# kwea123/nerf_pl

Hardware: AMD Instinct MI355X
Metric: rays/sec (64+128 samples), full training step: render_rays fwd + MSE + bwd + grad all-reduce + Adam (higher is better)
Workload: dtype bf16

## Files before the change

include/nerfhip.h:

```cpp
#ifndef NERFHIP_H
#define NERFHIP_H

#include <stddef.h>
#include <stdint.h>

#ifdef __cplusplus
extern "C" {
#endif

#define NERFHIP_ABI_VERSION 3

#define NERFHIP_E_BADARG (-1)
#define NERFHIP_E_UNSUPPORTED (-2)
#define NERFHIP_E_ALIGN (-3)
#define NERFHIP_E_DATA (-4)

#define NERFHIP_F32 0
#define NERFHIP_BF16 1
#define NERFHIP_BF16_F8 2

typedef void* nerfhip_stream_t;

int nerfhip_abi_version(void);
const char* nerfhip_error_string(int code);

int nerfhip_posenc(const float* x, float* out, int64_t n, int C, int n_freqs, nerfhip_stream_t stream);
int nerfhip_posenc_bwd(const float* x, const float* gout, float* gx, int64_t n, int C, int n_freqs,
                       nerfhip_stream_t stream);

int nerfhip_posenc_bands(const float* x, const float* bands, float* out, int64_t n, int C, int n_freqs,
                         nerfhip_stream_t stream);
int nerfhip_posenc_bands_bwd(const float* x, const float* bands, const float* gout, float* gx, int64_t n, int C, int n_freqs,
                             nerfhip_stream_t stream);

int nerfhip_sample_coarse_z(const float* rays, const float* perturb_rand, float* z, int64_t B, int S,
                            int use_disp, float perturb, nerfhip_stream_t stream);

int nerfhip_searchsorted_right(const float* a, const float* v, int64_t* idx, int64_t B, int M, int K,
                               nerfhip_stream_t stream);
int nerfhip_searchsorted_left(const float* a, const float* v, int64_t* idx, int64_t B, int M, int K,
                              nerfhip_stream_t stream);

int nerfhip_sample_pdf(const float* bins, int64_t bins_stride, const float* weights, int64_t w_stride,
                       const float* u, int64_t u_stride, float* samples, int64_t B, int M, int K, float eps,
                       nerfhip_stream_t stream);

#define NERFHIP_ROW_TOTAL_EXACT 0
#define NERFHIP_ROW_TOTAL_ATEN 1

int nerfhip_sample_pdf_ex(const float* bins, int64_t bins_stride, const float* weights, int64_t w_stride,
                          const float* u, int64_t u_stride, float* samples, int64_t B, int M, int K, float eps,
                          float* cdf_out, int64_t* inds_out, int row_total, nerfhip_stream_t stream);

int nerfhip_fine_z(const float* z_coarse, const float* w_coarse, const float* u, int64_t u_stride,
                   float* z_fine, float* z_new, int64_t B, int S_c, int N_i, float eps,
                   nerfhip_stream_t stream);

int nerfhip_fine_z_ex(const float* z_coarse, const float* w_coarse, const float* u, int64_t u_stride, float* z_fine,
                      float* z_new, int64_t B, int S_c, int N_i, float eps, float* cdf_out, int64_t* inds_out,
                      int row_total, nerfhip_stream_t stream);

int nerfhip_composite_fwd(const float* raw, int raw_ch, const float* z, const float* rays,
                          const float* noise, float noise_std, int white_back, float* weights, float* rgb,
                          float* depth, float* opacity, int64_t B, int S, nerfhip_stream_t stream);
int nerfhip_composite_bwd(const float* raw, int raw_ch, const float* z, const float* rays,
                          const float* noise, float noise_std, int white_back, const float* g_rgb,
                          const float* g_depth, const float* g_opacity, const float* g_weights,
                          float* g_raw, int64_t B, int S, nerfhip_stream_t stream);

int nerfhip_composite_train(const float* raw, const float* z, const float* rays, const float* noise, float noise_std,
                            int white_back, const float* target, float grad_scale, float* weights, float* rgb, float* depth,
                            float* opacity, float* g_raw, int64_t B, int S, nerfhip_stream_t stream);

int nerfhip_composite_train_fine_z(const float* raw, const float* z, const float* rays, const float* noise, float noise_std,
                                   int white_back, const float* target, float grad_scale, float* weights, float* rgb, float* depth,
                                   float* opacity, float* g_raw, int64_t B, int S, const float* u, int64_t u_stride, int N_i,
                                   float eps, float* z_fine, int row_total, nerfhip_stream_t stream);
int nerfhip_composite_train_loss(const float* raw, const float* z, const float* rays, const float* noise, float noise_std,
                                 int white_back, const float* target, float grad_scale, float* weights, float* rgb, float* depth,
                                 float* opacity, float* g_raw, int64_t B, int S, const float* rgb_coarse, float* out3,
                                 uint32_t* ticket, nerfhip_stream_t stream);

size_t nerfhip_mlp_packed_bytes(int dtype);
int nerfhip_mlp_pack_weights(const float* const* weights_host, const float* const* biases_host, void* packed,
                             int dtype, nerfhip_stream_t stream);

size_t nerfhip_mlp_act_bytes(int64_t n_points, int dtype);

int nerfhip_mlp_fwd_embedded(const float* x, int64_t x_stride, int64_t n, const void* packed, float* out,
                             int sigma_only, int dtype, void* save_acts, nerfhip_stream_t stream);

int nerfhip_mlp_fwd_rays(const float* rays, const float* z, int64_t B, int S, const void* packed, float* out,
                         int sigma_only, int dtype, void* save_acts, nerfhip_stream_t stream);

int nerfhip_mlp_fwd_rays_coarse(const float* rays, const float* perturb_rand, float* z, int64_t B, int S, int use_disp,
                                float perturb, const void* packed, float* out, int sigma_only, int dtype, void* save_acts,
                                nerfhip_stream_t stream);

size_t nerfhip_mlp_packed_bwd_bytes(int dtype);
int nerfhip_mlp_pack_weights_bwd(const float* const* weights_host, const float* const* biases_host, void* packed_bwd, int dtype,
                                 nerfhip_stream_t stream);
int nerfhip_mlp_pack_weights_train(const float* const* weights_host, const float* const* biases_host, void* packed,
                                   void* packed_bwd, int dtype, nerfhip_stream_t stream);
int nerfhip_mlp_pack_weights_train_multi(const float* const* weights_host, const float* const* biases_host,
                                         void* const* packed_host, void* const* packed_bwd_host, int n_models, int dtype,
                                         nerfhip_stream_t stream);
size_t nerfhip_mlp_dy_bytes(int64_t n_points, int dtype);
int nerfhip_mlp_dw_splits(int64_t n_points, int dtype);
size_t nerfhip_mlp_dw_workspace_bytes(int64_t n_points, int dtype);
int nerfhip_mlp_bwd(const float* g_out, const float* out, int64_t n, const void* packed_bwd, const void* acts,
                    void* dys, void* dw_workspace, float* const* grad_w_host, float* const* grad_b_host,
                    int accumulate, int dtype, nerfhip_stream_t stream);

int nerfhip_mlp_bwd_phases(const float* g_out, const float* out, int64_t n, const void* packed_bwd, const void* acts,
                           void* dys, void* dw_workspace, float* const* grad_w_host, float* const* grad_b_host,
                           int accumulate, int dtype, int phases, nerfhip_stream_t stream);

typedef struct nerfhip_adam_fused {
    int n_models;
    float* param[2];
    float* exp_avg[2];
    float* exp_avg_sq[2];
    const float* grad_flat[2];
    float* state;
    float lr, beta1, beta2, eps, weight_decay;
} nerfhip_adam_fused;
size_t nerfhip_mlp_dw_workspace_bytes_multi(const int64_t* n_points_host, int n_models, int dtype);
int nerfhip_mlp_dw_plan(const int64_t* n_points_host, int n_models, int dtype, int* splits_out, int* stage_kib_out);
int nerfhip_mlp_bwd_multi(int n_models, const float* const* g_out_host, const float* const* out_host, const int64_t* n_host,
                          const void* const* packed_bwd_host, const void* const* acts_host, void* const* dys_host,
                          void* dw_workspace, float* const* grad_w_host, float* const* grad_b_host, int accumulate, int dtype,
                          int phases, const float* g_scale, const nerfhip_adam_fused* adam, nerfhip_stream_t stream);

typedef struct nerfhip_enc_source {
    const float* rays[2];
    const float* z[2];
    int S[2];
} nerfhip_enc_source;
int nerfhip_mlp_bwd_multi_rays(int n_models, const float* const* g_out_host, const float* const* out_host, const int64_t* n_host,
                               const void* const* packed_bwd_host, const void* const* acts_host, void* const* dys_host,
                               void* dw_workspace, float* const* grad_w_host, float* const* grad_b_host, int accumulate, int dtype,
                               int phases, const float* g_scale, const nerfhip_adam_fused* adam, const nerfhip_enc_source* enc,
                               nerfhip_stream_t stream);

int nerfhip_mlp_dx_embedded(const void* dys, int64_t n, const float* w_xyz1, const float* w_xyz5, const float* w_dir,
                            float* gx, int64_t gx_stride, int dtype, nerfhip_stream_t stream);

#define NERFHIP_ACT_NONE 0
#define NERFHIP_ACT_RELU 1
#define NERFHIP_ACT_SIGMOID 2
int nerfhip_linear_fwd(const float* x, int64_t ldx, const float* w, int64_t ldw, const float* bias, float* y, int64_t ldy,
                       int64_t n, int n_in, int n_out, int act, int accumulate, int dtype, nerfhip_stream_t stream);
int nerfhip_linear_bwd_input(const float* gy, int64_t ldgy, const float* y, int64_t ldy, int act, const float* w, int64_t ldw,
                             float* gx, int64_t ldgx, int64_t n, int n_in, int n_out, int accumulate, int dtype,
                             nerfhip_stream_t stream);
size_t nerfhip_linear_bwd_weight_workspace_bytes(int64_t n, int n_in, int n_out);
int nerfhip_linear_bwd_weight(const float* gy, int64_t ldgy, const float* y, int64_t ldy, int act, const float* x, int64_t ldx,
                              float* gw, int64_t ldgw, float* gb, void* workspace, int64_t n, int n_in, int n_out,
                              int accumulate, int dtype, nerfhip_stream_t stream);

int nerfhip_mse_psnr(const float* rgb_coarse, const float* rgb_fine, const float* target, int64_t n, float* out3,
                     float* g_coarse, float* g_fine, nerfhip_stream_t stream);

int nerfhip_adam_step(float* const* params_host, const float* const* grads_host, float* const* exp_avg_host,
                      float* const* exp_avg_sq_host, const int64_t* numel_host, int n_tensors, float* state, float lr,
                      float beta1, float beta2, float eps, float weight_decay, nerfhip_stream_t stream);

int nerfhip_radam_step(float* const* params_host, const float* const* grads_host, float* const* exp_avg_host,
                       float* const* exp_avg_sq_host, const int64_t* numel_host, int n_tensors, float* state, double lr,
                       double beta1, double beta2, double eps, double weight_decay, int degenerated_to_sgd,
                       nerfhip_stream_t stream);
int nerfhip_ranger_step(float* const* params_host, const float* const* grads_host, float* const* exp_avg_host,
                        float* const* exp_avg_sq_host, const int64_t* numel_host, int n_tensors, float* state,
                        float* const* slow_host, double alpha, int k, double n_sma_threshold, double lr, double beta1,
                        double beta2, double eps, double weight_decay, nerfhip_stream_t stream);

int nerfhip_ray_directions(float* dirs, int H, int W, double focal, nerfhip_stream_t stream);
int nerfhip_get_rays(const float* directions, const float* c2w, float* rays_o, float* rays_d, int64_t n,
                     nerfhip_stream_t stream);
int nerfhip_ndc_rays(int H, int W, double focal, float near, const float* rays_o, const float* rays_d, float* out_o,
                     float* out_d, int64_t n, nerfhip_stream_t stream);
int nerfhip_gen_rays(const float* c2w, const int64_t* pixel_ids, int64_t first_pixel, int64_t n, int H, int W,
                     double focal, float near, float far, int use_ndc, float ndc_near_plane, float* rays,
                     nerfhip_stream_t stream);
int nerfhip_sample_batch(const float* c2w, const int64_t* pixel_ids, const float* rgbs_all, int64_t n, int H, int W,
                         double focal, float near, float far, int use_ndc, float ndc_near_plane, float* rays, float* rgbs,
                         nerfhip_stream_t stream);

#define NERFHIP_DRAW_UNIFORM 0
#define NERFHIP_DRAW_NORMAL 1
#define NERFHIP_DRAW_RANDINT 2
typedef struct nerfhip_draw {
    int kind;
    int64_t numel;
    void* out;
    uint64_t range;
} nerfhip_draw;
typedef struct nerfhip_ray_batch {
    const float* c2w;
    const float* rgbs_all;
    float* rays;
    float* rgbs;
    int H, W;
    double focal;
    float near, far;
    int use_ndc;
    float ndc_near_plane;
} nerfhip_ray_batch;
uint64_t nerfhip_torch_draw_increment(int64_t numel, int max_blocks);
int nerfhip_torch_draws(const nerfhip_draw* draws_host, int n_draws, const nerfhip_ray_batch* batch_host, uint64_t seed,
                        uint64_t offset, uint64_t* state, int max_blocks, uint64_t* increment_host, nerfhip_stream_t stream);

int nerfhip_train_prologue(const nerfhip_draw* draws_host, int n_draws, const nerfhip_ray_batch* batch_host, uint64_t seed,
                           uint64_t offset, uint64_t* state, int max_blocks, uint64_t* increment_host,
                           const float* const* weights_host, const float* const* biases_host, void* const* packed_host,
                           void* const* packed_bwd_host, int n_models, int dtype, nerfhip_stream_t stream);

typedef struct nerfhip_render_args {
    const float* rays;
    int64_t B;
    int S_c, N_i;
    const void* packed_coarse;
    const void* packed_fine;
    float* z_coarse;
    float* raw_coarse;
    float* z_fine;
    float* raw_fine;
    void* save_coarse;
    void* save_fine;
    const float* perturb_rand;
    float perturb;
    int use_disp;
    const float* noise_coarse;
    const float* noise_fine;
    float noise_std;
    int white_back;
    const float* u;
    int64_t u_stride;
    float eps;
    int row_total;
    float* rgb_coarse;
    float* depth_coarse;
    float* opacity_coarse;
    float* rgb_fine;
    float* depth_fine;
    float* opacity_fine;
    const float* target;
    float grad_scale;
    float* g_raw_coarse;
    float* g_raw_fine;
    float* out3;
    uint32_t* ticket;
    int regen_enc;
} nerfhip_render_args;
int nerfhip_render_supported(int64_t B, int S_c, int N_i, int dtype);
int nerfhip_render_fwd(const nerfhip_render_args* args_host, int dtype, nerfhip_stream_t stream);
int nerfhip_render_test_fwd(const nerfhip_render_args* args_host, int dtype, nerfhip_stream_t stream);
int nerfhip_render_train_fwd(const nerfhip_render_args* args_host, int dtype, nerfhip_stream_t stream);

size_t nerfhip_marching_cubes_workspace_bytes(int64_t n0, int64_t n1, int64_t n2);
int nerfhip_marching_cubes_count(const float* volume, int64_t n0, int64_t n1, int64_t n2, double iso, void* workspace,
                                 int64_t* totals, nerfhip_stream_t stream);
int nerfhip_marching_cubes_emit(const float* volume, int64_t n0, int64_t n1, int64_t n2, double iso, void* workspace,
                                const int64_t* totals, double* vertices, int32_t* triangles, nerfhip_stream_t stream);

int nerfhip_mesh_edge_keys(const int32_t* triangles, int64_t T, int64_t* keys, nerfhip_stream_t stream);
size_t nerfhip_mesh_cluster_workspace_bytes(int64_t V, int64_t T);
int nerfhip_mesh_largest_cluster(const int32_t* triangles, int64_t V, int64_t T, const int64_t* sorted_keys, const int64_t* order,
                                 void* workspace, int64_t* totals, nerfhip_stream_t stream);
int nerfhip_mesh_cluster_compact(const int32_t* triangles, int64_t V, int64_t T, void* workspace, int64_t* kept_vertex_ids,
                                 int32_t* kept_triangles, nerfhip_stream_t stream);

int nerfhip_mesh_vertex_normals(const float* vertices, int64_t V, const int32_t* triangles, int64_t T, double* normals,
                                nerfhip_stream_t stream);
int nerfhip_mesh_normal_rays(const float* vertices, const double* normals, int64_t V, float near, float far, float near_t,
                             float* rays, nerfhip_stream_t stream);
int nerfhip_mesh_view_rays(const float* vertices, int64_t V, const float* w2c_host, const float* origin_host, float focal, int W,
                           int H, const uint8_t* image, float near, uint8_t* colors, double* depth, float* rays,
                           nerfhip_stream_t stream);
int nerfhip_mesh_color_accumulate(const uint8_t* colors, const double* depth, const float* opacity, int64_t V,
                                  float occ_threshold, double* accum, nerfhip_stream_t stream);
int nerfhip_mesh_color_finish(const double* accum, int64_t V, uint8_t* out, nerfhip_stream_t stream);
int nerfhip_mesh_rgb_to_u8(const float* rgb, int64_t n, uint8_t* out, nerfhip_stream_t stream);

size_t nerfhip_vol_workspace_bytes(int64_t n);
int nerfhip_vol_pack(const float* rgbsigma, int64_t n, int64_t first_index, float neg_cell, void* workspace, uint32_t* records,
                     int64_t capacity, int64_t* cursor, nerfhip_stream_t stream);

int nerfhip_png_unfilter(const uint8_t* streams, uint8_t* out, int32_t* error_flags, int n_images, int H, int W, int ch,
                         nerfhip_stream_t stream);
int nerfhip_resize_rgba_lanczos(const uint8_t* in, uint8_t* out, uint8_t* workspace, int n_images, int in_h, int in_w, int out_h,
                                int out_w, const int32_t* xmin_h, const int32_t* count_h, const int32_t* taps_h, int ksize_h,
                                const int32_t* xmin_v, const int32_t* count_v, const int32_t* taps_v, int ksize_v,
                                nerfhip_stream_t stream);
int nerfhip_rgba_to_rgb_white(const uint8_t* rgba, float* rgb, uint8_t* valid_mask, int64_t n, nerfhip_stream_t stream);

int nerfhip_jpeg_entropy_decode(const uint8_t* scan, int64_t scan_bytes, int n_comp, const int32_t* comp, const uint8_t* huffman,
                                int huffman_mask, int mcus_x, int mcus_y, int restart_interval, int16_t* const* coef,
                                const int64_t* coef_blocks);
size_t nerfhip_jpeg_planes_bytes(int H, int W, int n_comp, int hs, int vs);
int nerfhip_jpeg_decode(const int16_t* coef_y, const int16_t* coef_cb, const int16_t* coef_cr, const uint16_t* quant,
                        uint8_t* planes, uint8_t* out, int n_images, int H, int W, int n_comp, int hs, int vs,
                        nerfhip_stream_t stream);

#define NERFHIP_IMAGE_PLANAR 0
#define NERFHIP_IMAGE_INTERLEAVED 1
size_t nerfhip_ssim_workspace_bytes(int B, int C, int H, int W);
int nerfhip_ssim(const float* img1, const float* img2, int B, int C, int H, int W, int window_size, int layout, float* map,
                 float* mean, void* workspace, nerfhip_stream_t stream);
size_t nerfhip_depth_colormap_workspace_bytes(int64_t n);
int nerfhip_depth_colormap(const float* depth, int64_t n, const uint8_t* table, float* out_chw, uint8_t* out_hwc, void* workspace,
                           nerfhip_stream_t stream);

#define NERFHIP_GIF_STRIP 3838
size_t nerfhip_gif_workspace_bytes(int F, int H, int W);
size_t nerfhip_gif_data_stride(int H, int W);
int nerfhip_gif_quantize(const uint8_t* frames, int F, int H, int W, uint8_t* indices, uint8_t* palettes, int32_t* box_counts,
                         void* workspace, nerfhip_stream_t stream);
int nerfhip_gif_lzw(const uint8_t* indices, int F, int H, int W, uint8_t* data, int32_t* lengths, void* workspace,
                    nerfhip_stream_t stream);

#define NERFHIP_PNG_STRIP 8192
size_t nerfhip_png_workspace_bytes(int n, int64_t stream_bytes);
size_t nerfhip_png_data_stride(int64_t stream_bytes);
int nerfhip_png_filter(const uint8_t* images, int n, int H, int W, int C, uint8_t* streams, nerfhip_stream_t stream);
int nerfhip_png_deflate(const uint8_t* streams, int n, int64_t stream_bytes, uint8_t* data, int32_t* lengths, uint32_t* adler,
                        void* workspace, nerfhip_stream_t stream);
int nerfhip_png_code_lengths(const uint32_t* counts, int n_symbols, int limit, uint8_t* lengths);

#ifdef __cplusplus
}
#endif
#endif
```

nerf_pl_amd/_lib.py:

```python
import ctypes
import functools
import os

import torch

_PKG = os.path.dirname(os.path.abspath(__file__))
LIB_PATH = os.environ.get("NERFHIP_LIB_PATH") or os.path.join(_PKG, "libnerfhip.so")

F32, BF16, BF16_F8 = 0, 1, 2

_c_void_p = ctypes.c_void_p
_i64 = ctypes.c_int64
_int = ctypes.c_int
_f32 = ctypes.c_float
_f64 = ctypes.c_double

SIGNATURES = {
    "nerfhip_abi_version": [],
    "nerfhip_error_string": [_int],
    "nerfhip_posenc": [_c_void_p, _c_void_p, _i64, _int, _int, _c_void_p],
    "nerfhip_posenc_bwd": [_c_void_p, _c_void_p, _c_void_p, _i64, _int, _int, _c_void_p],
    "nerfhip_posenc_bands": [_c_void_p, _c_void_p, _c_void_p, _i64, _int, _int, _c_void_p],
    "nerfhip_posenc_bands_bwd": [_c_void_p, _c_void_p, _c_void_p, _c_void_p, _i64, _int, _int, _c_void_p],
    "nerfhip_sample_coarse_z": [_c_void_p, _c_void_p, _c_void_p, _i64, _int, _int, _f32, _c_void_p],
    "nerfhip_searchsorted_right": [_c_void_p, _c_void_p, _c_void_p, _i64, _int, _int, _c_void_p],
    "nerfhip_searchsorted_left": [_c_void_p, _c_void_p, _c_void_p, _i64, _int, _int, _c_void_p],
    "nerfhip_sample_pdf": [_c_void_p, _i64, _c_void_p, _i64, _c_void_p, _i64, _c_void_p, _i64, _int, _int, _f32,
                           _c_void_p],
    "nerfhip_sample_pdf_ex": [_c_void_p, _i64, _c_void_p, _i64, _c_void_p, _i64, _c_void_p, _i64, _int, _int, _f32,
                              _c_void_p, _c_void_p, _int, _c_void_p],
    "nerfhip_fine_z_ex": [_c_void_p, _c_void_p, _c_void_p, _i64, _c_void_p, _c_void_p, _i64, _int, _int, _f32,
                          _c_void_p, _c_void_p, _int, _c_void_p],
    "nerfhip_fine_z": [_c_void_p, _c_void_p, _c_void_p, _i64, _c_void_p, _c_void_p, _i64, _int, _int, _f32,
                       _c_void_p],
    "nerfhip_composite_fwd": [_c_void_p, _int, _c_void_p, _c_void_p, _c_void_p, _f32, _int, _c_void_p, _c_void_p,
                              _c_void_p, _c_void_p, _i64, _int, _c_void_p],
    "nerfhip_composite_bwd": [_c_void_p, _int, _c_void_p, _c_void_p, _c_void_p, _f32, _int, _c_void_p, _c_void_p,
                              _c_void_p, _c_void_p, _c_void_p, _i64, _int, _c_void_p],
    "nerfhip_mlp_packed_bytes": [_int],
    "nerfhip_mlp_pack_weights": [ctypes.POINTER(_c_void_p), ctypes.POINTER(_c_void_p), _c_void_p, _int, _c_void_p],
    "nerfhip_mlp_act_bytes": [_i64, _int],
    "nerfhip_mlp_fwd_embedded": [_c_void_p, _i64, _i64, _c_void_p, _c_void_p, _int, _int, _c_void_p, _c_void_p],
    "nerfhip_mlp_fwd_rays": [_c_void_p, _c_void_p, _i64, _int, _c_void_p, _c_void_p, _int, _int, _c_void_p, _c_void_p],
    "nerfhip_mlp_packed_bwd_bytes": [_int],
    "nerfhip_mlp_pack_weights_bwd": [ctypes.POINTER(_c_void_p), ctypes.POINTER(_c_void_p), _c_void_p, _int, _c_void_p],
    "nerfhip_mlp_pack_weights_train": [ctypes.POINTER(_c_void_p), ctypes.POINTER(_c_void_p), _c_void_p, _c_void_p, _int, _c_void_p],
    "nerfhip_mlp_dy_bytes": [_i64, _int],
    "nerfhip_mlp_dw_splits": [_i64, _int],
    "nerfhip_mlp_dw_workspace_bytes": [_i64, _int],
    "nerfhip_ray_directions": [_c_void_p, _int, _int, ctypes.c_double, _c_void_p],
    "nerfhip_get_rays": [_c_void_p, _c_void_p, _c_void_p, _c_void_p, _i64, _c_void_p],
    "nerfhip_ndc_rays": [_int, _int, ctypes.c_double, _f32, _c_void_p, _c_void_p, _c_void_p, _c_void_p, _i64, _c_void_p],
    "nerfhip_gen_rays": [_c_void_p, _c_void_p, _i64, _i64, _int, _int, ctypes.c_double, _f32, _f32, _int, _f32, _c_void_p,
                         _c_void_p],
    "nerfhip_mse_psnr": [_c_void_p, _c_void_p, _c_void_p, _i64, _c_void_p, _c_void_p, _c_void_p, _c_void_p],
    "nerfhip_mlp_bwd_phases": [_c_void_p, _c_void_p, _i64, _c_void_p, _c_void_p, _c_void_p, _c_void_p,
                               ctypes.POINTER(_c_void_p), ctypes.POINTER(_c_void_p), _int, _int, _int, _c_void_p],
    "nerfhip_mlp_dx_embedded": [_c_void_p, _i64, _c_void_p, _c_void_p, _c_void_p, _c_void_p, _i64, _int, _c_void_p],
    "nerfhip_adam_step": [ctypes.POINTER(_c_void_p), ctypes.POINTER(_c_void_p), ctypes.POINTER(_c_void_p),
                          ctypes.POINTER(_c_void_p), ctypes.POINTER(_i64), _int, _c_void_p, _f32, _f32, _f32, _f32, _f32, _c_void_p],
    "nerfhip_radam_step": [ctypes.POINTER(_c_void_p), ctypes.POINTER(_c_void_p), ctypes.POINTER(_c_void_p),
                           ctypes.POINTER(_c_void_p), ctypes.POINTER(_i64), _int, _c_void_p, _f64, _f64, _f64, _f64, _f64, _int, _c_void_p],
    "nerfhip_ranger_step": [ctypes.POINTER(_c_void_p), ctypes.POINTER(_c_void_p), ctypes.POINTER(_c_void_p),
                            ctypes.POINTER(_c_void_p), ctypes.POINTER(_i64), _int, _c_void_p, ctypes.POINTER(_c_void_p), _f64, _int,
                            _f64, _f64, _f64, _f64, _f64, _f64, _c_void_p],
    "nerfhip_mlp_bwd": [_c_void_p, _c_void_p, _i64, _c_void_p, _c_void_p, _c_void_p, _c_void_p,
                        ctypes.POINTER(_c_void_p), ctypes.POINTER(_c_void_p), _int, _int, _c_void_p],
    "nerfhip_sample_batch": [_c_void_p, _c_void_p, _c_void_p, _i64, _int, _int, ctypes.c_double, _f32, _f32, _int, _f32, _c_void_p,
                             _c_void_p, _c_void_p],
    "nerfhip_mlp_pack_weights_train_multi": [ctypes.POINTER(_c_void_p), ctypes.POINTER(_c_void_p), ctypes.POINTER(_c_void_p),
                                             ctypes.POINTER(_c_void_p), _int, _int, _c_void_p],
    "nerfhip_render_supported": [_i64, _int, _int, _int],
    "nerfhip_render_test_fwd": [_c_void_p, _int, _c_void_p],
    "nerfhip_render_fwd": [_c_void_p, _int, _c_void_p],
    "nerfhip_render_train_fwd": [_c_void_p, _int, _c_void_p],
    "nerfhip_composite_train": [_c_void_p, _c_void_p, _c_void_p, _c_void_p, _f32, _int, _c_void_p, _f32, _c_void_p, _c_void_p,
                                _c_void_p, _c_void_p, _c_void_p, _i64, _int, _c_void_p],
    "nerfhip_composite_train_fine_z": [_c_void_p, _c_void_p, _c_void_p, _c_void_p, _f32, _int, _c_void_p, _f32, _c_void_p, _c_void_p,
                                       _c_void_p, _c_void_p, _c_void_p, _i64, _int, _c_void_p, _i64, _int, _f32, _c_void_p, _int, _c_void_p],
    "nerfhip_composite_train_loss": [_c_void_p, _c_void_p, _c_void_p, _c_void_p, _f32, _int, _c_void_p, _f32, _c_void_p, _c_void_p,
                                     _c_void_p, _c_void_p, _c_void_p, _i64, _int, _c_void_p, _c_void_p, _c_void_p, _c_void_p],
    "nerfhip_mlp_fwd_rays_coarse": [_c_void_p, _c_void_p, _c_void_p, _i64, _int, _int, _f32, _c_void_p, _c_void_p, _int, _int,
                                    _c_void_p, _c_void_p],
    "nerfhip_torch_draw_increment": [_i64, _int],
    "nerfhip_torch_draws": [_c_void_p, _int, _c_void_p, ctypes.c_uint64, ctypes.c_uint64, _c_void_p, _int,
                            ctypes.POINTER(ctypes.c_uint64), _c_void_p],
    "nerfhip_train_prologue": [_c_void_p, _int, _c_void_p, ctypes.c_uint64, ctypes.c_uint64, _c_void_p, _int,
                               ctypes.POINTER(ctypes.c_uint64), ctypes.POINTER(_c_void_p), ctypes.POINTER(_c_void_p),
                               ctypes.POINTER(_c_void_p), ctypes.POINTER(_c_void_p), _int, _int, _c_void_p],
    "nerfhip_mlp_dw_workspace_bytes_multi": [ctypes.POINTER(_i64), _int, _int],
    "nerfhip_mlp_dw_plan": [ctypes.POINTER(_i64), _int, _int, ctypes.POINTER(_int), ctypes.POINTER(_int)],
    "nerfhip_mlp_bwd_multi": [_int, ctypes.POINTER(_c_void_p), ctypes.POINTER(_c_void_p), ctypes.POINTER(_i64),
                              ctypes.POINTER(_c_void_p), ctypes.POINTER(_c_void_p), ctypes.POINTER(_c_void_p), _c_void_p,
                              ctypes.POINTER(_c_void_p), ctypes.POINTER(_c_void_p), _int, _int, _int, _c_void_p, _c_void_p, _c_void_p],
    "nerfhip_mlp_bwd_multi_rays": [_int, ctypes.POINTER(_c_void_p), ctypes.POINTER(_c_void_p), ctypes.POINTER(_i64),
                                   ctypes.POINTER(_c_void_p), ctypes.POINTER(_c_void_p), ctypes.POINTER(_c_void_p), _c_void_p,
                                   ctypes.POINTER(_c_void_p), ctypes.POINTER(_c_void_p), _int, _int, _int, _c_void_p, _c_void_p, _c_void_p,
                                   _c_void_p],
    "nerfhip_linear_fwd": [_c_void_p, _i64, _c_void_p, _i64, _c_void_p, _c_void_p, _i64, _i64, _int, _int, _int, _int, _int, _c_void_p],
    "nerfhip_linear_bwd_input": [_c_void_p, _i64, _c_void_p, _i64, _int, _c_void_p, _i64, _c_void_p, _i64, _i64, _int, _int, _int,
                                 _int, _c_void_p],
    "nerfhip_linear_bwd_weight_workspace_bytes": [_i64, _int, _int],
    "nerfhip_linear_bwd_weight": [_c_void_p, _i64, _c_void_p, _i64, _int, _c_void_p, _i64, _c_void_p, _i64, _c_void_p, _c_void_p,
                                  _i64, _int, _int, _int, _int, _c_void_p],
    "nerfhip_marching_cubes_workspace_bytes": [_i64, _i64, _i64],
    "nerfhip_marching_cubes_count": [_c_void_p, _i64, _i64, _i64, ctypes.c_double, _c_void_p, _c_void_p, _c_void_p],
    "nerfhip_marching_cubes_emit": [_c_void_p, _i64, _i64, _i64, ctypes.c_double, _c_void_p, _c_void_p, _c_void_p, _c_void_p,
                                    _c_void_p],
    "nerfhip_mesh_edge_keys": [_c_void_p, _i64, _c_void_p, _c_void_p],
    "nerfhip_mesh_cluster_workspace_bytes": [_i64, _i64],
    "nerfhip_mesh_largest_cluster": [_c_void_p, _i64, _i64, _c_void_p, _c_void_p, _c_void_p, _c_void_p, _c_void_p],
    "nerfhip_mesh_cluster_compact": [_c_void_p, _i64, _i64, _c_void_p, _c_void_p, _c_void_p, _c_void_p],
    "nerfhip_mesh_vertex_normals": [_c_void_p, _i64, _c_void_p, _i64, _c_void_p, _c_void_p],
    "nerfhip_mesh_normal_rays": [_c_void_p, _c_void_p, _i64, _f32, _f32, _f32, _c_void_p, _c_void_p],
    "nerfhip_mesh_view_rays": [_c_void_p, _i64, ctypes.POINTER(_f32), ctypes.POINTER(_f32), _f32, _int, _int, _c_void_p, _f32,
                               _c_void_p, _c_void_p, _c_void_p, _c_void_p],
    "nerfhip_mesh_color_accumulate": [_c_void_p, _c_void_p, _c_void_p, _i64, _f32, _c_void_p, _c_void_p],
    "nerfhip_mesh_color_finish": [_c_void_p, _i64, _c_void_p, _c_void_p],
    "nerfhip_mesh_rgb_to_u8": [_c_void_p, _i64, _c_void_p, _c_void_p],
    "nerfhip_vol_workspace_bytes": [_i64],
    "nerfhip_vol_pack": [_c_void_p, _i64, _i64, _f32, _c_void_p, _c_void_p, _i64, _c_void_p, _c_void_p],
    "nerfhip_png_unfilter": [_c_void_p, _c_void_p, _c_void_p, _int, _int, _int, _int, _c_void_p],
    "nerfhip_resize_rgba_lanczos": [_c_void_p, _c_void_p, _c_void_p, _int, _int, _int, _int, _int, _c_void_p, _c_void_p, _c_void_p,
                                    _int, _c_void_p, _c_void_p, _c_void_p, _int, _c_void_p],
    "nerfhip_rgba_to_rgb_white": [_c_void_p, _c_void_p, _c_void_p, _i64, _c_void_p],
    "nerfhip_jpeg_entropy_decode": [_c_void_p, _i64, _int, _c_void_p, _c_void_p, _int, _int, _int, _int, ctypes.POINTER(_c_void_p),
                                    ctypes.POINTER(_i64)],
    "nerfhip_jpeg_planes_bytes": [_int, _int, _int, _int, _int],
    "nerfhip_jpeg_decode": [_c_void_p, _c_void_p, _c_void_p, _c_void_p, _c_void_p, _c_void_p, _int, _int, _int, _int, _int, _int,
                            _c_void_p],
    "nerfhip_ssim_workspace_bytes": [_int, _int, _int, _int],
    "nerfhip_ssim": [_c_void_p, _c_void_p, _int, _int, _int, _int, _int, _int, _c_void_p, _c_void_p, _c_void_p, _c_void_p],
    "nerfhip_depth_colormap_workspace_bytes": [_i64],
    "nerfhip_depth_colormap": [_c_void_p, _i64, _c_void_p, _c_void_p, _c_void_p, _c_void_p, _c_void_p],
    "nerfhip_gif_workspace_bytes": [_int, _int, _int],
    "nerfhip_gif_data_stride": [_int, _int],
    "nerfhip_gif_quantize": [_c_void_p, _int, _int, _int, _c_void_p, _c_void_p, _c_void_p, _c_void_p, _c_void_p],
    "nerfhip_gif_lzw": [_c_void_p, _int, _int, _int, _c_void_p, _c_void_p, _c_void_p, _c_void_p],
    "nerfhip_png_workspace_bytes": [_int, _i64],
    "nerfhip_png_data_stride": [_i64],
    "nerfhip_png_filter": [_c_void_p, _int, _int, _int, _int, _c_void_p, _c_void_p],
    "nerfhip_png_deflate": [_c_void_p, _int, _i64, _c_void_p, _c_void_p, _c_void_p, _c_void_p, _c_void_p],
    "nerfhip_png_code_lengths": [_c_void_p, _int, _int, _c_void_p],
}


class AdamFused(ctypes.Structure):
    _fields_ = [("n_models", _int), ("param", _c_void_p * 2), ("exp_avg", _c_void_p * 2), ("exp_avg_sq", _c_void_p * 2),
                ("grad_flat", _c_void_p * 2), ("state", _c_void_p), ("lr", _f32), ("beta1", _f32), ("beta2", _f32), ("eps", _f32),
                ("weight_decay", _f32)]

class Draw(ctypes.Structure):
    _fields_ = [("kind", _int), ("numel", _i64), ("out", _c_void_p), ("range", ctypes.c_uint64)]


class RayBatch(ctypes.Structure):
    _fields_ = [("c2w", _c_void_p), ("rgbs_all", _c_void_p), ("rays", _c_void_p), ("rgbs", _c_void_p), ("H", _int), ("W", _int),
                ("focal", ctypes.c_double), ("near", _f32), ("far", _f32), ("use_ndc", _int), ("ndc_near_plane", _f32)]


class RenderArgs(ctypes.Structure):
    _fields_ = [("rays", _c_void_p), ("B", _i64), ("S_c", _int), ("N_i", _int), ("packed_coarse", _c_void_p), ("packed_fine", _c_void_p),
                ("z_coarse", _c_void_p), ("raw_coarse", _c_void_p), ("z_fine", _c_void_p), ("raw_fine", _c_void_p),
                ("save_coarse", _c_void_p), ("save_fine", _c_void_p), ("perturb_rand", _c_void_p), ("perturb", _f32), ("use_disp", _int),
                ("noise_coarse", _c_void_p), ("noise_fine", _c_void_p), ("noise_std", _f32), ("white_back", _int), ("u", _c_void_p),
                ("u_stride", _i64), ("eps", _f32), ("row_total", _int), ("rgb_coarse", _c_void_p), ("depth_coarse", _c_void_p),
                ("opacity_coarse", _c_void_p), ("rgb_fine", _c_void_p), ("depth_fine", _c_void_p), ("opacity_fine", _c_void_p),
                ("target", _c_void_p), ("grad_scale", _f32), ("g_raw_coarse", _c_void_p), ("g_raw_fine", _c_void_p), ("out3", _c_void_p),
                ("ticket", _c_void_p), ("regen_enc", _int)]


class EncSource(ctypes.Structure):
    _fields_ = [("rays", _c_void_p * 2), ("z", _c_void_p * 2), ("S", _int * 2)]


DRAW_UNIFORM, DRAW_NORMAL, DRAW_RANDINT = 0, 1, 2

_RESTYPES = {"nerfhip_error_string": ctypes.c_char_p, "nerfhip_torch_draw_increment": ctypes.c_uint64, "nerfhip_mlp_packed_bytes": ctypes.c_size_t,
             "nerfhip_mlp_act_bytes": ctypes.c_size_t, "nerfhip_mlp_packed_bwd_bytes": ctypes.c_size_t,
             "nerfhip_mlp_dy_bytes": ctypes.c_size_t, "nerfhip_mlp_dw_workspace_bytes": ctypes.c_size_t,
             "nerfhip_mlp_dw_workspace_bytes_multi": ctypes.c_size_t,
             "nerfhip_linear_bwd_weight_workspace_bytes": ctypes.c_size_t,
             "nerfhip_marching_cubes_workspace_bytes": ctypes.c_size_t, "nerfhip_mesh_cluster_workspace_bytes": ctypes.c_size_t,
             "nerfhip_jpeg_planes_bytes": ctypes.c_size_t, "nerfhip_ssim_workspace_bytes": ctypes.c_size_t,
             "nerfhip_depth_colormap_workspace_bytes": ctypes.c_size_t, "nerfhip_gif_workspace_bytes": ctypes.c_size_t,
             "nerfhip_gif_data_stride": ctypes.c_size_t, "nerfhip_vol_workspace_bytes": ctypes.c_size_t,
             "nerfhip_png_workspace_bytes": ctypes.c_size_t, "nerfhip_png_data_stride": ctypes.c_size_t}

_lib = None


class NerfHipError(RuntimeError):
    pass


def load():
    global _lib
    if _lib is not None:
        return _lib
    if not os.path.exists(LIB_PATH):
        raise NerfHipError(
            "libnerfhip.so not built: run `python -m nerf_pl_amd.build` (needs hipcc, gfx950). "
            "There is no CPU/eager fallback for the hot path.")
    lib = ctypes.CDLL(LIB_PATH, mode=ctypes.RTLD_GLOBAL)
    for name, argtypes in SIGNATURES.items():
        fn = getattr(lib, name)
        fn.argtypes = argtypes
        fn.restype = _RESTYPES.get(name, ctypes.c_int)
    if lib.nerfhip_abi_version() != 3:
        raise NerfHipError("libnerfhip ABI version mismatch")
    _lib = lib
    return lib


def check(code, what):
    if code != 0:
        msg = load().nerfhip_error_string(code)
        raise NerfHipError("%s failed: %s (code %d)" % (what, msg.decode() if msg else "?", code))


def stream_ptr():
    return ctypes.c_void_p(torch.cuda.current_stream().cuda_stream)


def _first_cuda_tensor(args):
    for a in args:
        if torch.is_tensor(a) and a.is_cuda:
            return a
        if isinstance(a, (list, tuple)):
            t = _first_cuda_tensor(a)
            if t is not None:
                return t
    return None


def device_guard(fn):
    @functools.wraps(fn)
    def wrapped(*args, **kw):
        t = _first_cuda_tensor(args)
        if t is None:
            t = _first_cuda_tensor(tuple(kw.values()))
        if t is None or t.device.index == torch.cuda.current_device():
            return fn(*args, **kw)
        with torch.cuda.device(t.device):
            return fn(*args, **kw)
    return wrapped


def ptr(t):
    if t is None:
        return None
    return ctypes.c_void_p(t.data_ptr())


def require_gpu(*tensors):
    dev = None
    for t in tensors:
        if t is None:
            continue
        if not t.is_cuda:
            raise NerfHipError("nerf_pl_amd runs on MI355X only: got a %s tensor (no CPU fallback)" % t.device)
        if t.dtype != torch.float32:
            raise NerfHipError("expected float32 tensor, got %s" % t.dtype)
        if dev is None:
            dev = t.device
        elif t.device != dev:
            raise NerfHipError("tensors of one call live on different GPUs (%s vs %s)" % (dev, t.device))
    if dev is not None and dev.index != torch.cuda.current_device():
        raise NerfHipError("launch on %s while the current device is cuda:%d (operator missing its device_guard)"
                           % (dev, torch.cuda.current_device()))
```

nerf_pl_amd/csrc/mlp_bwd.hip:

```cpp
#include "common.h"
#include "mlp_layout.h"
#include "mlp_bwd_chain.h"
#include "mlp_bwd_dw.h"
#include "mlp_dw_plan.h"

static_assert(kPlanF32 == NERFHIP_F32 && kPlanBf16 == NERFHIP_BF16 && kPlanBf16F8 == NERFHIP_BF16_F8, "mlp_dw_plan.h dtype codes");
static inline bool valid_dtype(int dtype) { return dtype == NERFHIP_F32 || dtype == NERFHIP_BF16 || dtype == NERFHIP_BF16_F8; }
static inline int compute_prec(int dtype) { return dtype == NERFHIP_F32 ? NERFHIP_F32 : NERFHIP_BF16; }
#if NERFHIP_DW_PROBE
static bool g_probe_f8 = false;
#endif

extern "C" size_t nerfhip_mlp_dy_bytes(int64_t n_points, int dtype) {
    if (n_points < 0 || !valid_dtype(dtype)) return 0;
    if (dtype == NERFHIP_BF16_F8) return (size_t)act_tiles(n_points, dtype) * nerfhip::mlp::f8_dy_tile_bytes();
    return (size_t)act_tiles(n_points, dtype) * nerfhip::mlp::kDySlabs * 64 * (dtype == NERFHIP_BF16 ? 16 : 32);
}

extern "C" int nerfhip_mlp_dw_splits(int64_t n_points, int dtype) {
    if (n_points <= 0 || !valid_dtype(dtype)) return 0;
    return dw_plan(&n_points, 1, dtype, nullptr);
}
static size_t dw_workspace_bytes(int nwg, int n_models) {
    return ((size_t)nwg * nerfhip::mlp::kDwSlabFloats + (size_t)n_models * nerfhip::mlp::kFoldScratchFloats) * sizeof(float);
}
extern "C" size_t nerfhip_mlp_dw_workspace_bytes(int64_t n_points, int dtype) {
    const int nwg = nerfhip_mlp_dw_splits(n_points, dtype);
    return nwg > 0 ? dw_workspace_bytes(nwg, 1) : 0;
}
extern "C" size_t nerfhip_mlp_dw_workspace_bytes_multi(const int64_t* n_points_host, int n_models, int dtype) {
    if (!n_points_host || n_models < 1 || n_models > nerfhip::kDwMaxModels || !valid_dtype(dtype)) return 0;
    for (int m = 0; m < n_models; ++m)
        if (n_points_host[m] <= 0) return 0;
    return dw_workspace_bytes(dw_plan(n_points_host, n_models, dtype, nullptr), n_models);
}

extern "C" int nerfhip_mlp_dw_plan(const int64_t* n_points_host, int n_models, int dtype, int* splits_out, int* stage_kib_out) {
    if (!n_points_host || !splits_out || n_models < 1 || n_models > nerfhip::kDwMaxModels || !valid_dtype(dtype)) return NERFHIP_E_BADARG;
    for (int m = 0; m < n_models; ++m)
        if (n_points_host[m] <= 0) return NERFHIP_E_BADARG;
    nerfhip::DwJobTable jt;
    const int total = dw_plan(n_points_host, n_models, dtype, &jt);
    for (int j = 0; j < n_models * nerfhip::mlp::kNumDwJobs; ++j) {
        splits_out[j] = jt.nsplit[j];
        if (stage_kib_out) {
            int slabs = jt.job[j].dy_slabs + jt.job[j].x1_slabs + jt.job[j].x2_slabs;
            if (jt.fold_of[j] >= 0 || jt.nsplit[j] == 0) slabs = 0;
            for (int k = 0; k < n_models * nerfhip::mlp::kNumDwJobs; ++k)
                if (jt.fold_of[k] == j) slabs += jt.job[k].dy_slabs;
            stage_kib_out[j] = dtype == NERFHIP_F32 ? 2 * slabs : slabs;
        }
    }
    return total;
}

extern "C" int nerfhip_mlp_bwd_multi(int n_models, const float* const* g_out_host, const float* const* out_host,
                                     const int64_t* n_host, const void* const* packed_bwd_host, const void* const* acts_host,
                                     void* const* dys_host, void* dw_workspace, float* const* grad_w_host,
                                     float* const* grad_b_host, int accumulate, int dtype, int phases, const float* g_scale,
                                     const nerfhip_adam_fused* adam, nerfhip_stream_t stream) {
    return nerfhip_mlp_bwd_multi_rays(n_models, g_out_host, out_host, n_host, packed_bwd_host, acts_host, dys_host, dw_workspace, grad_w_host,
                                      grad_b_host, accumulate, dtype, phases, g_scale, adam, nullptr, stream);
}

extern "C" int nerfhip_mlp_bwd_multi_rays(int n_models, const float* const* g_out_host, const float* const* out_host,
                                          const int64_t* n_host, const void* const* packed_bwd_host, const void* const* acts_host,
                                          void* const* dys_host, void* dw_workspace, float* const* grad_w_host,
                                          float* const* grad_b_host, int accumulate, int dtype, int phases, const float* g_scale,
                                          const nerfhip_adam_fused* adam, const nerfhip_enc_source* enc, nerfhip_stream_t stream) {
    NERFHIP_CHECK_ARG(n_models >= 1 && n_models <= nerfhip::kDwMaxModels);
    if (!valid_dtype(dtype)) return NERFHIP_E_UNSUPPORTED;
    bool regen[nerfhip::kDwMaxModels] = {false, false};
    if (enc) {
        if (dtype != NERFHIP_BF16) return NERFHIP_E_UNSUPPORTED;
        for (int m = 0; m < n_models; ++m) {
            if (!enc->rays[m]) continue;
            NERFHIP_CHECK_ARG(enc->z[m] && enc->S[m] > 0 && enc->S[m] % 32 == 0 && n_host[m] % 256 == 0 && n_host[m] % enc->S[m] == 0);
            NERFHIP_CHECK_ARG(n_host[m] / 32 < (int64_t)1 << 31);
            if ((((uintptr_t)enc->rays[m]) | ((uintptr_t)enc->z[m])) & 15) return NERFHIP_E_ALIGN;
            regen[m] = true;
        }
    }
    NERFHIP_CHECK_ARG(g_out_host && out_host && n_host && packed_bwd_host && acts_host && dys_host && grad_w_host && grad_b_host);
    NERFHIP_CHECK_ARG(!(adam && accumulate));
    nerfhip::GradTable G;
    nerfhip::DwJobTable jt;
    for (int m = 0; m < n_models; ++m) {
        NERFHIP_CHECK_ARG(n_host[m] > 0);
        NERFHIP_CHECK_ARG(g_out_host[m] && out_host[m] && packed_bwd_host[m] && acts_host[m] && dys_host[m] && dw_workspace);
        if ((((uintptr_t)g_out_host[m]) | ((uintptr_t)out_host[m]) | ((uintptr_t)packed_bwd_host[m]) | ((uintptr_t)acts_host[m]) |
             ((uintptr_t)dys_host[m])) & 15)
            return NERFHIP_E_ALIGN;
    }
    const int nwg = dw_plan(n_host, n_models, dtype, &jt);
    for (int m = 0; m < nerfhip::kDwMaxModels; ++m) {
        const bool on = m < n_models && regen[m];
        jt.enc_rays[m] = on ? enc->rays[m] : nullptr;
        jt.enc_z[m] = on ? enc->z[m] : nullptr;
        jt.enc_tpr[m] = on ? enc->S[m] / 32 : 1;
    }
    float* const fold_scratch = (float*)dw_workspace + (size_t)nwg * nerfhip::mlp::kDwSlabFloats;
    nerfhip::FoldArgs F;
    for (int m = 0; m < nerfhip::kDwMaxModels; ++m) {
        const int mm = m < n_models ? m : 0;
        F.image[m] = reinterpret_cast<const float*>((const uint8_t*)packed_bwd_host[mm] +
                                                    (size_t)nerfhip::mlp::bwd_padded_pieces(compute_prec(dtype)) * nerfhip::mlp::kPieceBytes);
        F.gw_final[m] = grad_w_host[12 * mm + 8];
        F.gb_final[m] = grad_b_host[12 * mm + 8];
        F.gw_dir[m] = grad_w_host[12 * mm + 9];
    }
    for (int j = 0; j < nerfhip::kDwMaxJobs; ++j) {
        const int jj = j < jt.njobs ? j : 0, m = jj / nerfhip::mlp::kNumDwJobs, prm = nerfhip::mlp::kDwJobs[jj % nerfhip::mlp::kNumDwJobs].param;
        NERFHIP_CHECK_ARG(grad_w_host[12 * m + prm] && grad_b_host[12 * m + prm]);
        G.w[j] = grad_w_host[12 * m + prm];
        G.b[j] = grad_b_host[12 * m + prm];
        jt.acts[j] = (const uint8_t*)acts_host[m];
        jt.dys[j] = (const uint8_t*)dys_host[m];
    }
    nerfhip::AdamFused A;
    A.state = nullptr;
    A.lr = A.beta1 = A.beta2 = A.eps = A.wd = 0.f;
    for (int m = 0; m < nerfhip::kDwMaxModels; ++m) { A.param[m] = A.m[m] = A.v[m] = nullptr; A.grad0[m] = nullptr; }
    if (adam) {
        NERFHIP_CHECK_ARG(adam->state && adam->n_models == n_models);
        for (int m = 0; m < n_models; ++m) {
            NERFHIP_CHECK_ARG(adam->param[m] && adam->exp_avg[m] && adam->exp_avg_sq[m] && adam->grad_flat[m]);
            A.param[m] = adam->param[m]; A.m[m] = adam->exp_avg[m]; A.v[m] = adam->exp_avg_sq[m]; A.grad0[m] = adam->grad_flat[m];
        }
        A.state = adam->state; A.lr = adam->lr; A.beta1 = adam->beta1; A.beta2 = adam->beta2; A.eps = adam->eps; A.wd = adam->weight_decay;
    }
    hipStream_t s = (hipStream_t)stream;
    const bool do_chain = phases & 1, do_dw = phases & 2, do_reduce = phases & 4;
    if (do_chain) {
        int64_t tiles[nerfhip::kDwMaxModels];
        for (int m = 0; m < n_models; ++m) tiles[m] = act_tiles(n_host[m], dtype);
        nerfhip::launch_bwd_chain(n_models, g_out_host, g_scale, out_host, n_host, packed_bwd_host, acts_host, dys_host, dtype, tiles, s);
    }
    if (do_dw) {
        if (dtype == NERFHIP_BF16_F8) nerfhip::launch_dw_f8(jt, (float*)dw_workspace, nwg, s);
        else nerfhip::launch_dw(dtype, jt, (float*)dw_workspace, nwg, s);
#if NERFHIP_DW_PROBE
        g_probe_f8 = dtype == NERFHIP_BF16_F8;
#endif
    }
    if (do_reduce) {
        nerfhip::launch_reduce(dtype == NERFHIP_BF16_F8, jt, (const float*)dw_workspace, G, fold_scratch, accumulate, A, s);
        nerfhip::launch_fold(F, (const float*)fold_scratch, n_models, accumulate, A, s);
    }
    return nerfhip_launch_status();
}

#if NERFHIP_DW_PROBE
extern "C" int nerfhip_debug_dw_probe(unsigned* host_dst, int n_words) {
    if (!host_dst || n_words < 0 || n_words > 1024 * 8 * 8) return NERFHIP_E_BADARG;
    return g_probe_f8 ? nerfhip::read_dw_f8_probe(host_dst, n_words) : nerfhip::read_dw_probe(host_dst, n_words);
}
#endif

extern "C" int nerfhip_mlp_bwd_phases(const float* g_out, const float* out, int64_t n, const void* packed_bwd, const void* acts,
                                      void* dys, void* dw_workspace, float* const* grad_w_host, float* const* grad_b_host,
                                      int accumulate, int dtype, int phases, nerfhip_stream_t stream) {
    NERFHIP_CHECK_ARG(n >= 0);
    if (!valid_dtype(dtype)) return NERFHIP_E_UNSUPPORTED;
    NERFHIP_CHECK_ARG(grad_w_host && grad_b_host);
    for (int i = 0; i < 12; ++i) NERFHIP_CHECK_ARG(grad_w_host[i] && grad_b_host[i]);
    if (n == 0) return 0;
    return nerfhip_mlp_bwd_multi(1, &g_out, &out, &n, &packed_bwd, &acts, &dys, dw_workspace, grad_w_host, grad_b_host, accumulate,
                                 dtype, phases, nullptr, nullptr, stream);
}

extern "C" int nerfhip_mlp_bwd(const float* g_out, const float* out, int64_t n, const void* packed_bwd, const void* acts,
                               void* dys, void* dw_workspace, float* const* grad_w_host, float* const* grad_b_host,
                               int accumulate, int dtype, nerfhip_stream_t stream) {
    return nerfhip_mlp_bwd_phases(g_out, out, n, packed_bwd, acts, dys, dw_workspace, grad_w_host, grad_b_host, accumulate, dtype, 7,
                                  stream);
}
```

nerf_pl_amd/csrc/mlp_bwd_chain.h:

```cpp
#pragma once
#include <hip/hip_runtime.h>
#include <stdint.h>

namespace nerfhip {
struct BwdChainArgs {
    const float* g_out[2];
    const float* out[2];
    int64_t n[2];
    const uint8_t* packed_bwd[2];
    const uint8_t* acts[2];
    uint8_t* dys[2];
    int blocks0;
};
void launch_bwd_chain(int n_models, const float* const* g_out, const float* g_scale, const float* const* out, const int64_t* n,
                      const void* const* packed_bwd, const void* const* acts, void* const* dys, int dtype, const int64_t* tiles,
                      hipStream_t s);
}
```

nerf_pl_amd/csrc/mlp_bwd_chain.hip:

```cpp
#include "mlp_device.h"
#include "f8_store.h"
#include "mlp_bwd_chain.h"

namespace nerfhip {

__device__ __forceinline__ float slab_absmax8(const bf16x8& s) {
    float m = 0.0f;
#pragma unroll
    for (int j = 0; j < 8; ++j) m = fmaxf(m, fabsf((float)s[j]));
    return m;
}
__device__ __forceinline__ float slab_absmax8(const f32x8& s) { return 0.0f; }

constexpr int kChainDepthBf16 = 2, kChainDepthF8 = 0;
constexpr int kChainBurst = 2;
template <int PREC> using BwdStream = RingStream<PrecTraits<PREC>::NW, bwd_chunks(PREC), true>;

template <typename Slab>
__device__ __forceinline__ Slab load_slab(__amdgpu_buffer_rsrc_t rsrc, int sec, int lane) {
    Slab s;
    u32x4* dst = reinterpret_cast<u32x4*>(&s);
    const unsigned voff = (unsigned)lane * (unsigned)sizeof(Slab);
    const unsigned soff = (unsigned)(sec * 64 * sizeof(Slab));
#pragma unroll
    for (int q = 0; q < (int)(sizeof(Slab) / 16); ++q) dst[q] = __builtin_amdgcn_raw_buffer_load_b128(rsrc, voff + 16 * q, soff, 0);
    return s;
}
template <int PREC, typename Slab>
__device__ __forceinline__ void store_slab(int& pending, __amdgpu_buffer_rsrc_t rsrc, int sec, const Slab& s, int lane) {
    const unsigned voff = (unsigned)lane * (unsigned)sizeof(Slab);
    const unsigned soff = (unsigned)(sec * 64 * sizeof(Slab) * act_il(PREC));
    store_slab_b128(pending, rsrc, s, voff + soff);
}

__device__ __forceinline__ void save_dy_pair(int& pending, uint8_t* dy_tile, int pair, const bf16x8& s0, const bf16x8& s1, int sb, int lane) {
    save_pair_bf8(pending, dy_tile, pair, s0, s1, sb, lane);
}
__device__ __forceinline__ void save_dy_pair(int&, uint8_t*, int, const f32x8&, const f32x8&, int, int) {}
__device__ __forceinline__ int dy_block_scale(float lane_max) { return bf8_block_scale(lane_max); }

template <int BIT>
__device__ __forceinline__ unsigned gate_mask(unsigned word) {
    unsigned m;
    asm("v_bfe_i32 %0, %1, %2, 1" : "=v"(m) : "v"(word), "n"(BIT));
    return m;
}

template <int PREC, int L, int NT, int NKS, bool MASK, bool F8, int IN_PAIRS, typename Slab>
__device__ __forceinline__ int run_bwd_layer_tm(BwdStream<PREC>& st, const unsigned lds_lo, const unsigned lds_hi, const unsigned sig_lds,
                                                const Slab (&gin)[NKS - kBwdLayers[L].sigma_slab], Slab* out,
                                                __amdgpu_buffer_rsrc_t acts, int gate_off, int mask_piece,
                                                __amdgpu_buffer_rsrc_t dys, uint8_t* dy_tile, int dy_sec, int dy_scale_idx, int in_sec,
                                                int in_sb, int lane) {
    constexpr int G0 = bwd_layer_start(L, PREC);
    constexpr int PPF = ppf(PREC);
    static_assert(kBwdLayers[L].nt == NT && kBwdLayers[L].nks == NKS, "bwd layer shape mismatch");
    auto piece_off = [](int g) { return ((g / kChunkPieces) % kSlots) * kChunkBytes + (g % kChunkPieces) * kPieceBytes; };
    typedef __attribute__((address_space(3))) const char* lds_cptr;
    auto piece_ptr = [&](int g) { return piece_off(g) < 65536 ? (lds_cptr)(lds_lo + (unsigned)piece_off(g)) : (lds_cptr)(lds_hi + (unsigned)(piece_off(g) - 65536)); };
    constexpr bool SIG = kBwdLayers[L].sigma_slab != 0;
    constexpr int NIN = NKS - (SIG ? 1 : 0);
    auto bslab = [&](int ks) -> Slab {
        if constexpr (SIG) {
            if (ks == NIN) return *reinterpret_cast<__attribute__((address_space(3))) const Slab*>(sig_lds);
        }
        return gin[ks < NIN ? ks : 0];
    };
    u32x4 gates = {0u, 0u, 0u, 0u};
    if (MASK)
        gates = __builtin_amdgcn_raw_buffer_load_b128(acts, (unsigned)lane * 16u, (unsigned)((gate_off + mask_piece * kPieceBytes) * act_il(PREC, F8)), 0);
    float mx = 0.0f;
    f32x16 acc2[2];
    constexpr int NFR = NT * NKS;
    constexpr int kChainDepth = F8 ? kChainDepthF8 : kChainDepthBf16;
    [[maybe_unused]] bf16x8 afr[kChainDepth > 0 ? kChainDepth : 1];
    [[maybe_unused]] auto frag_read = [&](auto ic) -> bf16x8 {
        constexpr int g = G0 + decltype(ic)::value * PPF;
        if constexpr (g % kChunkPieces == 0) st.boundary(g / kChunkPieces);
        return *reinterpret_cast<__attribute__((address_space(3))) const bf16x8*>(piece_ptr(g));
    };
    if constexpr (PREC == NERFHIP_BF16 && kChainDepth > 0) {
        static_for<0, (kChainDepth < NFR ? kChainDepth : NFR)>([&](auto jc) { afr[decltype(jc)::value] = frag_read(jc); });
    }
    static_for<0, NT>([&](auto tc) {
        constexpr int t = decltype(tc)::value;
        f32x16& acc = acc2[t & 1];
#pragma unroll
        for (int r = 0; r < 16; ++r) acc[r] = 0.0f;
        if constexpr (PREC == NERFHIP_BF16 && kChainDepth > 0) {
            static_for<0, NKS>([&](auto kc) {
                constexpr int ks = decltype(kc)::value;
                constexpr int i = t * NKS + ks;
                acc = __builtin_amdgcn_mfma_f32_32x32x16_bf16(afr[i % (kChainDepth > 0 ? kChainDepth : 1)], bslab(ks), acc, 0, 0, 0);
                if constexpr (i + kChainDepth < NFR) afr[i % (kChainDepth > 0 ? kChainDepth : 1)] = frag_read(std::integral_constant<int, i + kChainDepth>{});
                __builtin_amdgcn_sched_barrier(0);
            });
        } else {
#pragma unroll
        for (int ks = 0; ks < NKS; ++ks) {
            const int g = G0 + (t * NKS + ks) * PPF;
            if (g % kChunkPieces == 0) st.boundary(g / kChunkPieces);
            if constexpr (PREC == NERFHIP_BF16) {
                const bf16x8 a = *reinterpret_cast<__attribute__((address_space(3))) const bf16x8*>(piece_ptr(g));
                acc = __builtin_amdgcn_mfma_f32_32x32x16_bf16(a, bslab(ks), acc, 0, 0, 0);
            } else {
                const f32x4 a0 = *reinterpret_cast<__attribute__((address_space(3))) const f32x4*>(piece_ptr(g));
                if ((g + 1) % kChunkPieces == 0) st.boundary((g + 1) / kChunkPieces);
                const f32x4 a1 = *reinterpret_cast<__attribute__((address_space(3))) const f32x4*>(piece_ptr(g + 1));
                const Slab bs = bslab(ks);
#pragma unroll
                for (int j = 0; j < 4; ++j) acc = __builtin_amdgcn_mfma_f32_32x32x2f32(a0[j], bs[j], acc, 0, 0, 0);
#pragma unroll
                for (int j = 0; j < 4; ++j) acc = __builtin_amdgcn_mfma_f32_32x32x2f32(a1[j], bs[4 + j], acc, 0, 0, 0);
            }
        }
        }
        if constexpr (F8 && PREC == NERFHIP_BF16) {
            if constexpr (IN_PAIRS > 0) {
#pragma unroll
                for (int q = 0; q < IN_PAIRS; ++q)
                    if (q >= t * IN_PAIRS / NT && q < (t + 1) * IN_PAIRS / NT)
                        save_dy_pair(st.pending, dy_tile, in_sec / 2 + q, gin[2 * q], gin[2 * q + 1], in_sb, lane);
            }
        }
        if constexpr (PREC == NERFHIP_BF16 && MASK) {
            static_for<0, 8>([&](auto pc) {
                constexpr int p = decltype(pc)::value;
                constexpr int idx = 8 * (2 * t) + 2 * p;
                typedef __attribute__((ext_vector_type(2))) float f32x2v;
                typedef __attribute__((ext_vector_type(2))) __bf16 bf16x2q;
                typedef __attribute__((ext_vector_type(2))) short s16x2q;
                const f32x2v xv = {acc[2 * p], acc[2 * p + 1]};
                if (F8) mx = fmaxf(fmaxf(mx, fabsf(xv[0])), fabsf(xv[1]));
                const bf16x2q pk = __builtin_convertvector(xv, bf16x2q);
                const unsigned gword = gates[gate_word(idx)];
                s16x2q gm = __builtin_bit_cast(s16x2q, gword);
                gm = (gm << (short)((idx & 31) >> 1)) >> (short)15;
                const unsigned d = __builtin_bit_cast(unsigned, pk) & __builtin_bit_cast(unsigned, gm);
                const bf16x2q gated = __builtin_bit_cast(bf16x2q, d);
                out[2 * t + (p >> 2)][2 * (p & 3)] = gated[0];
                out[2 * t + (p >> 2)][2 * (p & 3) + 1] = gated[1];
            });
        } else {
        float v[16];
        static_for<0, 16>([&](auto rc) {
            constexpr int r = decltype(rc)::value;
            constexpr int idx = 8 * (2 * t) + r;
            const float gv = acc[r];
            if constexpr (MASK) v[r] = __uint_as_float(__float_as_uint(gv) & gate_mask<gate_bit(idx)>(gates[gate_word(idx)]));
            else v[r] = gv;
            if (F8) mx = fmaxf(mx, fabsf(v[r]));
        });
#pragma unroll
        for (int sl = 0; sl < 2; ++sl) {
            float v8[8];
#pragma unroll
            for (int j = 0; j < 8; ++j) v8[j] = v[8 * sl + j];
            make_slab(out[2 * t + sl], v8);
        }
        }
        if constexpr (!F8) {
            __amdgpu_buffer_rsrc_t dys_l = __builtin_amdgcn_make_buffer_rsrc(dy_tile + (size_t)dy_sec * 64 * sizeof(Slab) * act_il(PREC), 0,
                                                                              (int)(2 * NT * 64 * sizeof(Slab) * act_il(PREC)), 0x00020000);
            constexpr int TB = kChainBurst / 2 > 0 ? kChainBurst / 2 : 1;
            if constexpr ((t + 1) % TB == 0 || t == NT - 1) {
                constexpr int t0 = (t / TB) * TB;
#pragma unroll
                for (int sl = 2 * t0; sl < 2 * t + 2; ++sl) store_slab<PREC>(st.pending, dys_l, sl, out[sl], lane);
            }
        }
    });
    if constexpr (F8 && PREC == NERFHIP_BF16) {
        const int sb = dy_block_scale(mx);
        save_scale_f8(st.pending, dy_tile, f8_dy_scale_off(), dy_scale_idx, sb, lane);
        return sb;
    }
    return 127;
}

template <int PREC, bool F8>
__global__ __launch_bounds__(PrecTraits<PREC>::NW * 64, PrecTraits<PREC>::WPS)
void mlp_bwd_chain_kernel(BwdChainArgs A, const float* __restrict__ g_scale) {
    const int mdl = ((int)blockIdx.x >= A.blocks0) ? 1 : 0;
    const unsigned wg = blockIdx.x - (mdl ? (unsigned)A.blocks0 : 0u);
    const float* __restrict__ g_out = mdl ? A.g_out[1] : A.g_out[0];
    const float* __restrict__ out = mdl ? A.out[1] : A.out[0];
    const int64_t n = mdl ? A.n[1] : A.n[0];
    const uint8_t* __restrict__ packed_bwd = mdl ? A.packed_bwd[1] : A.packed_bwd[0];
    const uint8_t* __restrict__ acts_base = mdl ? A.acts[1] : A.acts[0];
    uint8_t* __restrict__ dys_base = mdl ? A.dys[1] : A.dys[0];
    static_assert(!F8 || PREC == NERFHIP_BF16, "fp8 storage is a bf16-compute mode");
    using Slab = typename PrecTraits<PREC>::Slab;
    constexpr int kActTile = F8 ? f8_act_tile_bytes() : act_tile_bytes(PREC);
    constexpr int kGateOff = F8 ? f8_act_gate_off() : act_mask_off(PREC);
    constexpr int kDyTile = F8 ? f8_dy_tile_bytes() : kDySlabs * 64 * (int)sizeof(Slab);
    constexpr int NW = PrecTraits<PREC>::NW;
    __shared__ __attribute__((aligned(1024))) char ring[kSlots * kChunkBytes + NW * 64 * (int)sizeof(Slab)];
#if NERFHIP_STREAM_PROBE
    const uint64_t probe_t0 = __builtin_amdgcn_s_memrealtime();
#endif
    const int lane = threadIdx.x & 63;
    const int wave = __builtin_amdgcn_readfirstlane((int)(threadIdx.x >> 6));
    const int h = lane >> 5;
    const int64_t tile = (int64_t)wg * NW + wave;
    const int64_t p = tile * 32 + (lane & 31);
    const bool valid = p < n;
    const int64_t pc = valid ? p : n - 1;

    float4 g = reinterpret_cast<const float4*>(g_out)[pc];
    const float4 o = reinterpret_cast<const float4*>(out)[pc];
    if (!valid) g = make_float4(0.f, 0.f, 0.f, 0.f);
    if (g_scale) {
        const float sc = *g_scale;
        g.x *= sc; g.y *= sc; g.z *= sc; g.w *= sc;
    }

    constexpr int IL = act_il(PREC, F8);
    __amdgpu_buffer_rsrc_t acts = __builtin_amdgcn_make_buffer_rsrc(
        const_cast<uint8_t*>(acts_base) + tile_block_off(tile, kActTile, IL), 0, kActTile * IL, 0x00020000);
    uint8_t* dy_tile = dys_base + tile_block_off(tile, kDyTile, IL);
    __amdgpu_buffer_rsrc_t dys = __builtin_amdgcn_make_buffer_rsrc(dy_tile, 0, kDyTile * IL, 0x00020000);


    BwdStream<PREC> st;
    st.gsrc = packed_bwd;
    st.voff = (unsigned)lane * 16u;
    st.lds_base = (unsigned)(uintptr_t)ring;
    st.wave = wave;
    st.pending = 0;
    st.pending_prev = 0;
    st.issue_chunk(0);
    st.issue_chunk(1);
    const unsigned lds_lo = (unsigned)(uintptr_t)ring + (unsigned)lane * 16u;
    unsigned lds_hi = lds_lo + 65536u;
    asm volatile("" : "+v"(lds_hi));
    const unsigned sig_lds = (unsigned)(uintptr_t)ring + (unsigned)(kSlots * kChunkBytes) + (unsigned)((wave * 64 + lane) * (int)sizeof(Slab));

    float v[8];
    Slab zero_slab;
#pragma unroll
    for (int j = 0; j < 8; ++j) v[j] = 0.0f;
    make_slab(zero_slab, v);
    Slab g_rgb, g_sig;
    {
        const float ga[3] = {g.x * o.x * (1.0f - o.x), g.y * o.y * (1.0f - o.y), g.z * o.z * (1.0f - o.z)};
#pragma unroll
        for (int j = 0; j < 8; ++j) v[j] = (h == 0 && j < 3) ? ga[j < 3 ? j : 0] : 0.0f;
        make_slab(g_rgb, v);
#pragma unroll
        for (int j = 0; j < 8; ++j) v[j] = (h == 0 && j == 0) ? g.w : 0.0f;
        make_slab(g_sig, v);
    }
    if constexpr (F8) {
        if constexpr (PREC == NERFHIP_BF16) {
            const int sb_rgb = bf8_block_scale(slab_absmax8(g_rgb)), sb_sig = bf8_block_scale(slab_absmax8(g_sig));
            save_pair_bf8(st.pending, dy_tile, kDyRgb / 2, g_rgb, zero_slab, sb_rgb, lane);
            save_pair_bf8(st.pending, dy_tile, kDySigma / 2, g_sig, zero_slab, sb_sig, lane);
            save_scale_f8(st.pending, dy_tile, f8_dy_scale_off(), f8_dy_section(kDyRgb), sb_rgb, lane);
            save_scale_f8(st.pending, dy_tile, f8_dy_scale_off(), f8_dy_section(kDySigma), sb_sig, lane);
        }
    } else {
        store_slab<PREC>(st.pending, dys, kDyRgb, g_rgb, lane);
        store_slab<PREC>(st.pending, dys, kDyRgb + 1, zero_slab, lane);
        store_slab<PREC>(st.pending, dys, kDySigma, g_sig, lane);
        store_slab<PREC>(st.pending, dys, kDySigma + 1, zero_slab, lane);
    }

    Slab gd[8];
    Slab ga[16], gb[16];
    Slab g_in0[1] = {g_rgb};
    int sb = run_bwd_layer_tm<PREC, 0, 4, 1, true, F8, 0>(st, lds_lo, lds_hi, sig_lds, g_in0, gd, acts, kGateOff, kMaskPieceT, dys, dy_tile, kDyDir,
                                                          f8_dy_section(kDyDir), -1, 127, lane);
    *reinterpret_cast<__attribute__((address_space(3))) Slab*>(sig_lds) = g_sig;
    static_assert(kBwdLayerFold == 1, "layer sequence below");
    sb = run_bwd_layer_tm<PREC, 1, 8, 9, true, F8, 4>(st, lds_lo, lds_hi, sig_lds, gd, gb, acts, kGateOff, mask_piece_h(8), dys, dy_tile, dy_h(8),
                                                      f8_dy_section(dy_h(8)), kDyDir, sb, lane);
    static_assert(bwd_layer_pieces(2, PREC) * 3 % (kChunkPieces * kSlots) == 0, "three looped layers = a whole number of ring turns");
#define NH_BWD(L, IN, OUT, D)                                                                                                \
    sb = run_bwd_layer_tm<PREC, L, 8, 16, true, F8, 8>(st, lds_lo, lds_hi, sig_lds, reinterpret_cast<const Slab(&)[16]>(IN), OUT, acts, kGateOff, \
                                                       mask_piece_h(9 - L) - (D), dys, dy_tile, dy_h(9 - L) + 16 * (D),              \
                                                       f8_dy_section(dy_h(9 - L)) + (D), dy_h(10 - L) + 16 * (D), sb, lane);
    if constexpr (PREC != NERFHIP_BF16) {
        NH_BWD(2, gb, ga, 0) NH_BWD(3, ga, gb, 0) NH_BWD(4, gb, ga, 0) NH_BWD(5, ga, gb, 0) NH_BWD(6, gb, ga, 0) NH_BWD(7, ga, gb, 0)
    } else {
        const uint8_t* const gsrc0 = st.gsrc;
        int n_pass;
        asm volatile("s_mov_b32 %0, 2" : "=s"(n_pass));
#pragma clang loop unroll(disable)
        for (int pass = 0; pass < n_pass; ++pass) {
            st.pending = 0;
            st.pending_prev = 0;
            const int d = 3 * pass;
            NH_BWD(2, gb, ga, d) NH_BWD(3, ga, gb, d) NH_BWD(4, gb, ga, d)
#pragma unroll
            for (int i = 0; i < 16; ++i) gb[i] = ga[i];
            st.gsrc += (size_t)(3 * bwd_layer_pieces(2, PREC)) * kPieceBytes;
        }
        st.pending = 0;
        st.pending_prev = 0;
        st.gsrc = gsrc0;
    }
    NH_BWD(8, gb, ga, 0)
#undef NH_BWD
    if constexpr (F8 && PREC == NERFHIP_BF16) {
#pragma unroll
        for (int q = 0; q < 8; ++q) save_dy_pair(st.pending, dy_tile, dy_h(1) / 2 + q, ga[2 * q], ga[2 * q + 1], sb, lane);
    }
#if NERFHIP_STREAM_PROBE
    if (lane == 0) {
        unsigned* pr = reinterpret_cast<unsigned*>(dy_tile);
        pr[0] = st.pr_wait; pr[1] = st.pr_bar; pr[2] = st.pr_n;
        pr[3] = (unsigned)(__builtin_amdgcn_s_memrealtime() - probe_t0);
    }
#endif
}


}

namespace nerfhip {
void launch_bwd_chain(int n_models, const float* const* g_out, const float* g_scale, const float* const* out, const int64_t* n,
                      const void* const* packed_bwd, const void* const* acts, void* const* dys, int dtype, const int64_t* tiles,
                      hipStream_t s) {
    const int wpw = (dtype == NERFHIP_F32) ? 4 : 8;
    BwdChainArgs A;
    unsigned blocks = 0;
    for (int m = 0; m < 2; ++m) {
        const int mm = m < n_models ? m : 0;
        A.g_out[m] = g_out[mm]; A.out[m] = out[mm]; A.n[m] = n[mm];
        A.packed_bwd[m] = (const uint8_t*)packed_bwd[mm]; A.acts[m] = (const uint8_t*)acts[mm]; A.dys[m] = (uint8_t*)dys[mm];
        if (m == 0) A.blocks0 = (int)(tiles[0] / wpw);
        if (m < n_models) blocks += (unsigned)(tiles[m] / wpw);
    }
    if (dtype == NERFHIP_BF16_F8)
        hipLaunchKernelGGL((mlp_bwd_chain_kernel<NERFHIP_BF16, true>), dim3(blocks), dim3(512), 0, s, A, g_scale);
    else if (dtype == NERFHIP_BF16)
        hipLaunchKernelGGL((mlp_bwd_chain_kernel<NERFHIP_BF16, false>), dim3(blocks), dim3(512), 0, s, A, g_scale);
    else
        hipLaunchKernelGGL((mlp_bwd_chain_kernel<NERFHIP_F32, false>), dim3(blocks), dim3(256), 0, s, A, g_scale);
}
}
```

nerf_pl_amd/csrc/mlp_bwd_dw.h:

```cpp
#pragma once
#include <stdint.h>

#include "mlp_layout.h"

typedef struct ihipStream_t* hipStream_t;

#ifndef NERFHIP_DW_PROBE
#define NERFHIP_DW_PROBE 0
#endif

namespace nerfhip {
using namespace mlp;

constexpr int kDwMaxModels = 2;
constexpr int kDwMaxJobs = kDwMaxModels * kNumDwJobs;
struct DwJobTable {
    DwJob job[kDwMaxJobs];
    int nsplit[kDwMaxJobs];
    int soff[kDwMaxJobs + 1];
    const uint8_t* acts[kDwMaxJobs];
    const uint8_t* dys[kDwMaxJobs];
    int64_t ntiles[kDwMaxJobs];
    int njobs;
    int fold_of[kDwMaxJobs];
    const float* enc_rays[kDwMaxModels];
    const float* enc_z[kDwMaxModels];
    int enc_tpr[kDwMaxModels];
};
static_assert(kDwJobs[kDwJobDir].x2_off == kDwJobs[kDwJobSigma].x1_off && kDwJobs[kDwJobDir].x2_slabs == 16 && kDwJobs[kDwJobDir].x1_slabs == 2 &&
              kDwJobs[kDwJobSigma].x1_slabs == 16 && kDwJobs[kDwJobSigma].dy_slabs == 2 && kDwJobs[kDwJobDir].dy_slabs == 8 &&
              kDwJobs[kDwJobSigma].x2_slabs == 0, "the sigma head and the dir layer read the same h8 section");
constexpr int kDwFoldRow0 = 4;
NH_HD constexpr int dw_fold_block(int xt) { return (kDwFoldRow0 + xt / 2) * kDwMaxXTiles + (xt & 1); }
constexpr int kDwFoldStageSlabs = 28;
constexpr int kDwFoldSigmaSlab = 26;

struct GradTable {
    float* w[kDwMaxJobs];
    float* b[kDwMaxJobs];
};

struct AdamFused {
    float* param[kDwMaxModels];
    float* m[kDwMaxModels];
    float* v[kDwMaxModels];
    const float* grad0[kDwMaxModels];
    float* state;
    float lr, beta1, beta2, eps, wd;
};

struct FoldArgs {
    const float* image[kDwMaxModels];
    float* gw_final[kDwMaxModels];
    float* gb_final[kDwMaxModels];
    float* gw_dir[kDwMaxModels];
};

void launch_dw(int prec, const DwJobTable& jt, float* slabs, int nwg, hipStream_t s);
void launch_dw_f8(const DwJobTable& jt, float* slabs, int nwg, hipStream_t s);
void launch_reduce(bool f8, const DwJobTable& jt, const float* slabs, const GradTable& G, float* fold_scratch, int accumulate,
                   const AdamFused& A, hipStream_t s);
void launch_fold(const FoldArgs& F, const float* fold_scratch, int n_models, int accumulate, const AdamFused& A, hipStream_t s);
#if NERFHIP_DW_PROBE
int read_dw_probe(unsigned* host_dst, int n_words);
int read_dw_f8_probe(unsigned* host_dst, int n_words);
#endif
}
```

nerf_pl_amd/csrc/mlp_bwd_dw.hip:

```cpp
#include "mlp_device.h"
#include "mlp_bwd_dw.h"

namespace nerfhip {

#if NERFHIP_DW_PROBE
__device__ unsigned g_dw_probe[1024 * 8 * 8];
#endif

constexpr int kDwRingKiB = 160, kDwMaxDepth = 12;
constexpr int kDwFragRing = 5, kDwFragRing2D = 4;

template <int PREC> struct DwTraits;
template <> struct DwTraits<NERFHIP_BF16> {
    static constexpr int SPP = 1;
    static constexpr int RING_BYTES = kDwRingKiB * 1024;
    static constexpr int DEPTH = 0, STAGE_BYTES = 0;
};
template <> struct DwTraits<NERFHIP_F32> {
    static constexpr int SPP = 2;
    static constexpr int DEPTH = 2;
    static constexpr int MAXP = 72;
    static constexpr int STAGE_BYTES = MAXP * kPieceBytes;
    static constexpr int RING_BYTES = DEPTH * STAGE_BYTES;
};

template <int PREC> NH_HD constexpr int dw_depth(int pieces) {
    if (PREC != NERFHIP_BF16) return DwTraits<PREC>::DEPTH;
    const int d = DwTraits<PREC>::RING_BYTES / (pieces * kPieceBytes);
    return d > kDwMaxDepth ? kDwMaxDepth : d;
}

__device__ __forceinline__ void dw_bias_sum(const bf16x8& a, float& s0, float& s1) {
    const bf16x2 one = {(__bf16)1.0f, (__bf16)1.0f};
    s0 = __builtin_amdgcn_fdot2_f32_bf16(bf16x2{a[0], a[1]}, one, s0, false);
    s1 = __builtin_amdgcn_fdot2_f32_bf16(bf16x2{a[2], a[3]}, one, s1, false);
    s0 = __builtin_amdgcn_fdot2_f32_bf16(bf16x2{a[4], a[5]}, one, s0, false);
    s1 = __builtin_amdgcn_fdot2_f32_bf16(bf16x2{a[6], a[7]}, one, s1, false);
}

template <int F, int SLABS>
__device__ __forceinline__ bf16x8 dw_encode_slab(const float (&v)[3], int h, int ks) {
    constexpr int NPAIR = 3 * (F / 2);
    constexpr float kInv2PiHi = 0.15915494f, kInv2PiLo = 6.4206297e-9f;
    float rh[3], rl[3];
#pragma unroll
    for (int c = 0; c < 3; ++c) {
        const float vs = h ? 2.0f * v[c] : v[c];
        rh[c] = vs * kInv2PiHi;
        rl[c] = __builtin_fmaf(vs, kInv2PiHi, -rh[c]) + vs * kInv2PiLo;
    }
    bf16x8 out;
#pragma unroll
    for (int q = 0; q < 4; ++q) {
        const int p = 4 * ks + q;
        float s, co;
        if (p < NPAIR) {
            const int i = p / 3, c = p - 3 * i;
            const float sc = (float)(1 << (2 * i));
            const float rhc = c == 0 ? rh[0] : (c == 1 ? rh[1] : rh[2]), rlc = c == 0 ? rl[0] : (c == 1 ? rl[1] : rl[2]);
            const float t = __builtin_amdgcn_fractf(rhc * sc) + rlc * sc;
            s = __builtin_amdgcn_sinf(t);
            co = __builtin_amdgcn_cosf(t);
        } else {
            const int tail = 2 * (p - NPAIR);
            s = (tail == 0) ? (h ? v[2] : v[0]) : 0.0f;
            co = (tail == 0) ? (h ? 0.0f : v[1]) : 0.0f;
        }
        out[2 * q] = (__bf16)s;
        out[2 * q + 1] = (__bf16)co;
    }
    return out;
}

template <int PREC>
__global__ __launch_bounds__(512, 2)
void mlp_bwd_dw_kernel(DwJobTable jobs, float* __restrict__ slabs) {
    constexpr int SPP = DwTraits<PREC>::SPP;
    constexpr int SLAB_BYTES = SPP * kPieceBytes;
    constexpr int IL = act_il(PREC);
    constexpr int RING_BYTES = DwTraits<PREC>::RING_BYTES;
    __shared__ __attribute__((aligned(1024))) char ring[RING_BYTES];

    const int lane = threadIdx.x & 63;
    const int wave = __builtin_amdgcn_readfirstlane((int)(threadIdx.x >> 6));
    int jid = 0;
#pragma unroll
    for (int j = 1; j < kDwMaxJobs; ++j) jid += ((int)blockIdx.x >= jobs.soff[j]) ? 1 : 0;
    const int nsplit = jobs.nsplit[jid], split = (int)blockIdx.x - jobs.soff[jid];
    const DwJob jb = jobs.job[jid];
    const int64_t ntiles = jobs.ntiles[jid];
    const uint8_t* __restrict__ acts_base = jobs.acts[jid];
    const uint8_t* __restrict__ dys_base = jobs.dys[jid];
    [[maybe_unused]] const float* __restrict__ enc_rays = jobs.enc_rays[jid / kNumDwJobs];
    [[maybe_unused]] const float* __restrict__ enc_z = jobs.enc_z[jid / kNumDwJobs];
    [[maybe_unused]] const int enc_tpr = jobs.enc_tpr[jid / kNumDwJobs];
    const int n_ot = jb.dy_slabs / 2;
    const int n_xs = jb.x1_slabs + jb.x2_slabs;
    const int n_xt = n_xs / 2;
    const int64_t per = (ntiles + nsplit - 1) / nsplit;
    const int64_t t_first = (int64_t)split * per;
    const int64_t my_tiles = (t_first >= ntiles) ? 0 : ((ntiles - t_first < per) ? ntiles - t_first : per);
    const unsigned lds_base = (unsigned)(uintptr_t)ring;

    const int dma_off_even = (PREC == NERFHIP_BF16) ? ((lane & 1) * 32 + (lane >> 1)) * 16 : lane * 16;
    const int dma_off_odd = (PREC == NERFHIP_BF16) ? ((lane & 1) * 32 + ((lane ^ 8) >> 1)) * 16 : lane * 16;

    f32x16 acc[kDwMaxXTiles];
#pragma unroll
    for (int x = 0; x < kDwMaxXTiles; ++x)
#pragma unroll
        for (int r = 0; r < 16; ++r) acc[x][r] = 0.0f;
    float dbacc = 0.0f;
    [[maybe_unused]] float dbacc2 = 0.0f;

    const int grp = lane >> 4, c = lane & 15;
    const int tr_off = (grp & 1) * SLAB_BYTES + (2 * (8 * (grp >> 1) + (c >> 2)) + ((c & 3) & 1)) * 16 + ((c & 3) >> 1) * 8;
    const int tr_s0 = (grp & 1) ? 128 : 0, tr_s1 = 128 - tr_s0;
    [[maybe_unused]] auto load_frag = [&](const char* pb, int q) { return load_frag_tr16(pb, tr_off, tr_s0, tr_s1, q); };
    const int m32 = lane & 31, kk = lane >> 5;
    const int f32_off = (m32 >> 4) * SLAB_BYTES + (slab_nat_h(m32 & 15) * 32) * 32 + slab_nat_j(m32 & 15) * 4;
#if NERFHIP_DW_PROBE
    unsigned pr_wait = 0, pr_bar = 0, pr_issue = 0, pr_comp = 0, pr_depth = 0;
    const uint64_t pr_t00 = __builtin_amdgcn_s_memrealtime();
#endif

    auto run = [&](auto nxt_c, auto nsl_c, auto regen_c) {
        constexpr int NXT = decltype(nxt_c)::value, NSL = decltype(nsl_c)::value;
        constexpr bool REGEN = decltype(regen_c)::value;
        static_assert(!REGEN || (PREC == NERFHIP_BF16 && (NXT == 2 || NXT == 9 || NXT == 10)), "classes with an encoding section");
        constexpr int ENC = REGEN ? (NXT == 9 ? kDirSlabs : kXyzSlabs) : 0;
        constexpr int DYS = NXT == 9 ? 8 : 16;
        constexpr bool FOLD = NXT == 9 && NSL == kDwFoldStageSlabs;
        constexpr bool SPLIT2D = (PREC == NERFHIP_BF16) && (NXT == 8 || NXT == 10) && (NSL - 2 * NXT >= 16);
        constexpr int NP = NSL * SPP;
        constexpr int NPD = NP - ENC;
        constexpr int LPWD = (NPD + 7) / 8;
        constexpr int LPW = LPWD + (REGEN ? 1 : 0);
        constexpr int STAGE = (PREC == NERFHIP_BF16) ? NP * kPieceBytes : DwTraits<PREC>::STAGE_BYTES;
        constexpr int ZSLOT = 256;
        constexpr int D0 = dw_depth<PREC>(NP);
        constexpr int D = (REGEN && D0 * (STAGE + ZSLOT) > RING_BYTES) ? D0 - 1 : D0;
        static_assert(D >= 2 && D * (STAGE + (REGEN ? ZSLOT : 0)) <= RING_BYTES, "ring stages of this job class");
        static_assert((D - 2) * LPW <= 63, "counted vmcnt");
#if NERFHIP_DW_PROBE
        pr_depth = D;
#endif
        int s_issue = 0, s_use = 0;
        const uint8_t* abase = nullptr;
        const uint8_t* dbase = nullptr;
        unsigned slot = 0;
        auto stage_tile = [&](int64_t it) {
            int64_t T = t_first + (it < my_tiles ? it : my_tiles - 1);
            if (T >= ntiles) T = ntiles - 1;
            return T;
        };
        const float* zsrc = nullptr;
        unsigned zslot = 0;
        int z_issue = 0, g_slot = 0;
        const unsigned lds_z = lds_base + (unsigned)(D * STAGE);
        auto next_z = [&](int64_t st) {
            zsrc = enc_z + stage_tile(st) * 32 + (lane & 31);
            zslot = (unsigned)__builtin_amdgcn_readfirstlane((int)(lds_z + (unsigned)(z_issue * ZSLOT)));
            z_issue = (z_issue + 1 == D) ? 0 : z_issue + 1;
        };
        auto next_stage = [&](int64_t it) {
            const int64_t T = stage_tile(it);
            abase = acts_base + tile_block_off(T, act_tile_bytes(PREC), IL);
            dbase = dys_base + tile_block_off(T, kDySlabs * 64 * (16 * SPP), IL);
            slot = lds_base + (unsigned)(s_issue * STAGE);
            s_issue = (s_issue + 1 == D) ? 0 : s_issue + 1;
            if constexpr (REGEN) next_z(it + 1);
        };
        float ray_next[6] = {0.f, 0.f, 0.f, 0.f, 0.f, 0.f};
        auto load_ray = [&](int64_t st) {
            if (wave < ENC) {
                const unsigned r = (unsigned)__builtin_amdgcn_readfirstlane((int)((unsigned)stage_tile(st) / (unsigned)enc_tpr));
                typedef const float __attribute__((address_space(4))) * ConstF;
                const ConstF rp = (ConstF)(uintptr_t)(enc_rays + (size_t)r * 8);
#pragma unroll
                for (int c = 0; c < 6; ++c) ray_next[c] = rp[c];
            }
        };
        auto gen_stage = [&](int64_t st) {
            if (wave < ENC) {
                const int n = lane & 31, h = lane >> 5;
                bf16x8 e;
                if constexpr (NXT == 9) {
                    const float dv[3] = {ray_next[3], ray_next[4], ray_next[5]};
                    e = dw_encode_slab<4, kDirSlabs>(dv, h, wave);
                } else {
                    const float zv = *reinterpret_cast<const float*>(ring + D * STAGE + g_slot * ZSLOT + n * 4);
                    float xv[3];
#pragma unroll
                    for (int c = 0; c < 3; ++c) xv[c] = nh_add(ray_next[c], nh_mul(ray_next[3 + c], zv));
                    e = dw_encode_slab<10, kXyzSlabs>(xv, h, wave);
                }
                const int unit = (2 * n + h) ^ ((wave & 1) ? 8 : 0);
                *reinterpret_cast<bf16x8*>(ring + g_slot * STAGE + (DYS + wave) * SLAB_BYTES + unit * 16) = e;
            }
            g_slot = (g_slot + 1 == D) ? 0 : g_slot + 1;
            load_ray(st + 1);
        };
        constexpr int REM = NPD % 8;
        constexpr bool SHARE_LAST = (PREC == NERFHIP_BF16) && (REM == 4 || REM == 2);
        const int share_piece = NPD - REM + (SHARE_LAST ? (wave * REM) / 8 : 0);
        const unsigned long long share_mask = REM == 4 ? (0xffffffffull << (32 * (wave & 1))) : (0xffffull << (16 * (wave & 3)));
        auto issue_piece = [&](int i) {
            if constexpr (REGEN) {
                if (i == LPW - 1) {
                    glds4(zsrc, zslot);
                    return;
                }
            }
            int pi = wave + 8 * i;
            const bool shared = SHARE_LAST && i == LPWD - 1;
            if (shared) pi = share_piece;
            if (pi >= NPD) pi = NPD - 1;
            if (REGEN && pi >= DYS) pi += ENC;
            const int sl = pi / SPP, sub = pi % SPP;
            const uint8_t* src;
            if (FOLD && sl >= kDwFoldSigmaSlab) src = dbase + (size_t)(kDySigma + sl - kDwFoldSigmaSlab) * 64 * (16 * SPP) * IL;
            else if (sl < jb.dy_slabs) src = dbase + (size_t)(jb.dy_off + sl) * 64 * (16 * SPP) * IL;
            else if (sl < jb.dy_slabs + jb.x1_slabs) src = abase + (size_t)(jb.x1_off + sl - jb.dy_slabs) * 64 * (16 * SPP) * IL;
            else src = abase + (size_t)(jb.x2_off + sl - jb.dy_slabs - jb.x1_slabs) * 64 * (16 * SPP) * IL;
            const uint8_t* g = src + (size_t)sub * kPieceBytes + ((sl & 1) ? dma_off_odd : dma_off_even);
            const unsigned dst = (unsigned)__builtin_amdgcn_readfirstlane((int)(slot + (unsigned)(pi * kPieceBytes)));
            if (shared) glds16_nt_masked(g, dst, share_mask);
            else glds16_nt(g, dst);
        };
        auto issue_stage = [&](int64_t it) {
            next_stage(it);
#pragma unroll
            for (int i = 0; i < LPW; ++i) issue_piece(i);
        };
        constexpr bool SPREAD = (PREC == NERFHIP_BF16);
        constexpr int DMA_STEP = (2 * NXT) / LPW > 0 ? (2 * NXT) / LPW : 1;
        if constexpr (REGEN) {
            next_z(0);
            glds4(zsrc, zslot);
            load_ray(0);
        }
#pragma unroll
        for (int s = 0; s < D - 1; ++s) issue_stage(s);
        if constexpr (REGEN) {
            wait_vm<(D - 1) * LPW>();
            gen_stage(0);
        }
        for (int64_t it = 0; it < my_tiles; ++it) {
#if NERFHIP_DW_PROBE
            const unsigned t0 = shader_cycles();
            wait_vm<(PREC == NERFHIP_BF16) ? (D - 2) * LPW : 0>();
            const unsigned t1 = shader_cycles();
            asm volatile("s_barrier" ::: "memory");
            const unsigned t2 = shader_cycles();
            pr_wait += (t1 - t0) & 0xffffffffu;
            pr_bar += (t2 - t1) & 0xffffffffu;
#else
            wait_vm_barrier<(PREC == NERFHIP_BF16) ? (D - 2) * LPW : 0>();
#endif
            if (SPREAD && (SPLIT2D || wave < n_ot)) next_stage(it + D - 1);
            else issue_stage(it + D - 1);
#if NERFHIP_DW_PROBE
            const unsigned t3 = shader_cycles();
            pr_issue += (t3 - t2) & 0xffffffffu;
#endif
            const char* st_base = ring + s_use * STAGE;
            s_use = (s_use + 1 == D) ? 0 : s_use + 1;
            if constexpr (SPLIT2D) {
                constexpr int XW = NXT / 2, NF = 2 * XW, RD = kDwFragRing2D;
                static_assert(RD >= 2 && RD <= NF, "B fragment ring");
                const int wi = wave >> 1, wj = wave & 1;
                const char* dyb = st_base + (4 * wi) * SLAB_BYTES;
                const char* x_all = st_base + 16 * SLAB_BYTES;
                const char* xb = x_all + (2 * XW * wj) * SLAB_BYTES;
                auto dma_after = [](int k) constexpr { return ((k + 1) * NF) / LPW - 1; };
                bf16x8 a[2][2], b[RD];
                a[0][0] = load_frag(dyb, 0);
                a[0][1] = load_frag(dyb + 2 * SLAB_BYTES, 0);
#pragma unroll
                for (int f = 0; f < RD - 1; ++f) b[f] = load_frag(xb + 2 * (f % XW) * SLAB_BYTES, f / XW);
                a[1][0] = load_frag(dyb, 1);
                a[1][1] = load_frag(dyb + 2 * SLAB_BYTES, 1);
                __builtin_amdgcn_sched_barrier(0);
#pragma unroll
                for (int f = 0; f < NF; ++f) {
                    if (f + RD - 1 < NF) b[(f + RD - 1) % RD] = load_frag(xb + 2 * ((f + RD - 1) % XW) * SLAB_BYTES, (f + RD - 1) / XW);
                    __builtin_amdgcn_sched_barrier(0);
                    acc[2 * (f % XW)] = __builtin_amdgcn_mfma_f32_32x32x16_bf16(a[f / XW][0], b[f % RD], acc[2 * (f % XW)], 0, 0, 0);
                    acc[2 * (f % XW) + 1] = __builtin_amdgcn_mfma_f32_32x32x16_bf16(a[f / XW][1], b[f % RD], acc[2 * (f % XW) + 1], 0, 0, 0);
                    __builtin_amdgcn_sched_barrier(0);
                    if (f == 0 || f == XW) {
                        const bf16x8 ab = wj ? a[f / XW][1] : a[f / XW][0];
                        dw_bias_sum(ab, dbacc, dbacc2);
                    }
                    if constexpr (SPREAD) {
#pragma unroll
                        for (int k = 0; k < LPW; ++k)
                            if (dma_after(k) == f) {
                                issue_piece(k);
                                __builtin_amdgcn_sched_barrier(0);
                            }
                    }
                }
            } else if (wave < n_ot) {
                const char* dy_base = st_base + (2 * wave) * SLAB_BYTES;
                const char* x_base = st_base + jb.dy_slabs * SLAB_BYTES;
                if constexpr (PREC == NERFHIP_BF16) {
                    constexpr int RD = kDwFragRing, NM = 2 * NXT;
                    const bf16x8 a0 = load_frag(dy_base, 0);
                    bf16x8 b[RD];
#pragma unroll
                    for (int m = 0; m < RD - 1; ++m)
                        if (m < NM) b[m] = load_frag(x_base + 2 * (m % NXT) * SLAB_BYTES, m / NXT);
                    const bf16x8 a1 = load_frag(dy_base, 1);
                    __builtin_amdgcn_sched_barrier(0);
#pragma unroll
                    for (int m = 0; m < NM; ++m) {
                        const int x = m % NXT;
                        if (m + RD - 1 < NM) b[(m + RD - 1) % RD] = load_frag(x_base + 2 * ((m + RD - 1) % NXT) * SLAB_BYTES, (m + RD - 1) / NXT);
                        __builtin_amdgcn_sched_barrier(0);
                        acc[x] = __builtin_amdgcn_mfma_f32_32x32x16_bf16(m < NXT ? a0 : a1, b[m % RD], acc[x], 0, 0, 0);
                        __builtin_amdgcn_sched_barrier(0);
                        if (m == 1) dw_bias_sum(a0, dbacc, dbacc2);
                        if (m == NXT + 1 || (NXT == 1 && m == 1)) dw_bias_sum(a1, dbacc, dbacc2);
                        if constexpr (SPREAD) {
                            if (m % DMA_STEP == DMA_STEP - 1 && m / DMA_STEP < LPW) {
                                issue_piece(m / DMA_STEP);
                                __builtin_amdgcn_sched_barrier(0);
                            }
                        }
                    }
                    if constexpr (SPREAD) {
#pragma unroll
                        for (int i = (2 * NXT) / DMA_STEP; i < LPW; ++i) issue_piece(i);
                    }
                } else {
#pragma unroll 4
                    for (int ks = 0; ks < 16; ++ks) {
                        const int pt = 2 * ks + kk;
                        const float a = *reinterpret_cast<const float*>(dy_base + f32_off + pt * 32);
                        dbacc += a;
#pragma unroll
                        for (int x = 0; x < NXT; ++x) {
                            const float b = *reinterpret_cast<const float*>(x_base + 2 * x * SLAB_BYTES + f32_off + pt * 32);
                            acc[x] = __builtin_amdgcn_mfma_f32_32x32x2f32(a, b, acc[x], 0, 0, 0);
                        }
                    }
                }
            } else if constexpr (FOLD) {
                const char* sg = st_base + kDwFoldSigmaSlab * SLAB_BYTES;
                const char* xs = st_base + (jb.dy_slabs + 2 * (1 + 2 * (wave - kDwFoldRow0))) * SLAB_BYTES;
                if constexpr (PREC == NERFHIP_BF16) {
                    const bf16x8 a0 = load_frag(sg, 0), b00 = load_frag(xs, 0), b10 = load_frag(xs + 2 * SLAB_BYTES, 0);
                    const bf16x8 a1 = load_frag(sg, 1), b01 = load_frag(xs, 1), b11 = load_frag(xs + 2 * SLAB_BYTES, 1);
                    acc[0] = __builtin_amdgcn_mfma_f32_32x32x16_bf16(a0, b00, acc[0], 0, 0, 0);
                    acc[1] = __builtin_amdgcn_mfma_f32_32x32x16_bf16(a0, b10, acc[1], 0, 0, 0);
                    acc[0] = __builtin_amdgcn_mfma_f32_32x32x16_bf16(a1, b01, acc[0], 0, 0, 0);
                    acc[1] = __builtin_amdgcn_mfma_f32_32x32x16_bf16(a1, b11, acc[1], 0, 0, 0);
                    if (wave == kDwFoldRow0) {
                        dw_bias_sum(a0, dbacc, dbacc2);
                        dw_bias_sum(a1, dbacc, dbacc2);
                    }
                } else {
#pragma unroll 4
                    for (int ks = 0; ks < 16; ++ks) {
                        const int pt = 2 * ks + kk;
                        const float a = *reinterpret_cast<const float*>(sg + f32_off + pt * 32);
                        dbacc += a;
                        const float b0 = *reinterpret_cast<const float*>(xs + f32_off + pt * 32);
                        const float b1 = *reinterpret_cast<const float*>(xs + 2 * SLAB_BYTES + f32_off + pt * 32);
                        acc[0] = __builtin_amdgcn_mfma_f32_32x32x2f32(a, b0, acc[0], 0, 0, 0);
                        acc[1] = __builtin_amdgcn_mfma_f32_32x32x2f32(a, b1, acc[1], 0, 0, 0);
                    }
                }
            }
            if constexpr (REGEN) gen_stage(it + 1);
#if NERFHIP_DW_PROBE
            pr_comp += (shader_cycles() - t3) & 0xffffffffu;
#endif
        }
        asm volatile("s_waitcnt vmcnt(0)" ::: "memory");
        float* sl = slabs + (size_t)blockIdx.x * kDwSlabFloats;
        dbacc += dbacc2;
        if constexpr (SPLIT2D) {
            constexpr int XW = NXT / 2;
            const int wi = wave >> 1, wj = wave & 1;
#pragma unroll
            for (int xl = 0; xl < XW; ++xl)
#pragma unroll
                for (int d = 0; d < 2; ++d)
                    dw_store_block(sl + (size_t)((2 * wi + d) * kDwMaxXTiles + XW * wj + xl) * 1024, acc[2 * xl + d], lane);
            sl[8 * kDwMaxXTiles * 64 * 16 + (2 * wi + wj) * 64 + lane] = dbacc;
        } else if (wave < n_ot) {
#pragma unroll
            for (int x = 0; x < NXT; ++x) dw_store_block(sl + (size_t)(wave * kDwMaxXTiles + x) * 1024, acc[x], lane);
            sl[8 * kDwMaxXTiles * 64 * 16 + wave * 64 + lane] = dbacc;
        } else if constexpr (FOLD) {
            dw_store_block(sl + (size_t)dw_fold_block(2 * (wave - kDwFoldRow0)) * 1024, acc[0], lane);
            dw_store_block(sl + (size_t)dw_fold_block(2 * (wave - kDwFoldRow0) + 1) * 1024, acc[1], lane);
            if (wave == kDwFoldRow0) sl[8 * kDwMaxXTiles * 64 * 16 + kDwFoldRow0 * 64 + lane] = dbacc;
        }
    };
    using std::integral_constant;
    using std::false_type;
    using std::true_type;
    bool regen = false;
    if constexpr (PREC == NERFHIP_BF16) regen = enc_rays != nullptr;
    switch (n_xt) {
        case 2:
            if constexpr (PREC == NERFHIP_BF16) {
                if (regen) { run(integral_constant<int, 2>{}, integral_constant<int, 20>{}, true_type{}); break; }
            }
            run(integral_constant<int, 2>{}, integral_constant<int, 20>{}, false_type{});
            break;
        case 4: run(integral_constant<int, 4>{}, integral_constant<int, 10>{}, false_type{}); break;
        case 8:
            if (jb.dy_slabs == 16) run(integral_constant<int, 8>{}, integral_constant<int, 32>{}, false_type{});
            else run(integral_constant<int, 8>{}, integral_constant<int, 18>{}, false_type{});
            break;
        case 9:
            if (jobs.fold_of[(jid / kNumDwJobs) * kNumDwJobs + kDwJobSigma] == jid) {
                if constexpr (PREC == NERFHIP_BF16) {
                    if (regen) { run(integral_constant<int, 9>{}, integral_constant<int, kDwFoldStageSlabs>{}, true_type{}); break; }
                }
                run(integral_constant<int, 9>{}, integral_constant<int, kDwFoldStageSlabs>{}, false_type{});
            } else {
                run(integral_constant<int, 9>{}, integral_constant<int, 26>{}, false_type{});
            }
            break;
        default:
            if constexpr (PREC == NERFHIP_BF16) {
                if (regen) { run(integral_constant<int, 10>{}, integral_constant<int, 36>{}, true_type{}); break; }
            }
            run(integral_constant<int, 10>{}, integral_constant<int, 36>{}, false_type{});
            break;
    }
#if NERFHIP_DW_PROBE
    if (lane == 0 && blockIdx.x < 1024) {
        unsigned* pr = g_dw_probe + ((size_t)blockIdx.x * 8 + wave) * 8;
        pr[0] = (unsigned)my_tiles; pr[1] = pr_wait; pr[2] = pr_bar; pr[3] = pr_issue; pr[4] = pr_comp;
        pr[5] = (unsigned)(__builtin_amdgcn_s_memrealtime() - pr_t00);
        pr[6] = (unsigned)jid; pr[7] = pr_depth;
    }
#endif
}

NH_HD constexpr bool dw_job_has_class(const DwJob& j) {
    const int nxt = (j.x1_slabs + j.x2_slabs) / 2, nsl = j.dy_slabs + j.x1_slabs + j.x2_slabs;
    return (nxt == 2 && nsl == 20) || (nxt == 4 && nsl == 10) || (nxt == 8 && ((nsl == 32 && j.dy_slabs == 16) || (nsl == 18 && j.dy_slabs != 16))) ||
           (nxt == 9 && nsl == 26) || (nxt == 10 && nsl == 36);
}
NH_HD constexpr bool dw_jobs_have_classes() {
    for (int j = 0; j < kNumDwJobs; ++j)
        if (!dw_job_has_class(kDwJobs[j])) return false;
    return true;
}
static_assert(dw_jobs_have_classes(), "mlp_bwd_dw_kernel: a weight-gradient job without a compiled job class");

void launch_dw(int prec, const DwJobTable& jt, float* slabs, int nwg, hipStream_t s) {
    if (prec == NERFHIP_BF16) hipLaunchKernelGGL(mlp_bwd_dw_kernel<NERFHIP_BF16>, dim3(nwg), dim3(512), 0, s, jt, slabs);
    else hipLaunchKernelGGL(mlp_bwd_dw_kernel<NERFHIP_F32>, dim3(nwg), dim3(512), 0, s, jt, slabs);
}
#if NERFHIP_DW_PROBE
int read_dw_probe(unsigned* host_dst, int n_words) {
    return hipMemcpyFromSymbol(host_dst, HIP_SYMBOL(g_dw_probe), (size_t)n_words * 4, 0, hipMemcpyDeviceToHost) == hipSuccess ? 0 : -100;
}
#endif

}
```

nerf_pl_amd/csrc/mlp_bwd_reduce.hip:

```cpp
#include "mlp_device.h"
#include "adam_math.h"
#include "mlp_bwd_dw.h"

namespace nerfhip {

struct GradEmit {
    const AdamFused& A;
    AdamCoef ac;
    int accumulate, model;
    __device__ __forceinline__ void operator()(float* dst, float val) const {
        const float g = accumulate ? *dst + val : val;
        *dst = g;
        if (A.state) {
            const size_t e = (size_t)(dst - A.grad0[model]);
            adam_elem(A.param[model][e], g, A.m[model][e], A.v[model][e], ac, A.beta2, A.eps, A.wd);
        }
    }
};

template <bool F8>
__global__ __launch_bounds__(256) void mlp_bwd_reduce_kernel(DwJobTable jobs, const float* __restrict__ slabs, GradTable G,
                                                              float* __restrict__ fold_scratch, int accumulate, AdamFused A) {
    const int jid = blockIdx.y;
    const DwJob jb = jobs.job[jid];
    const int model = jid / kNumDwJobs;
    const int fold = jobs.fold_of[jid];
    const int nsplit = jobs.nsplit[fold >= 0 ? fold : jid], s0 = jobs.soff[fold >= 0 ? fold : jid];
    const bool derived = jid % kNumDwJobs == kDwJobFinal;
    const int n_ot = derived ? 0 : jb.dy_slabs / 2, n_xt = (jb.x1_slabs + jb.x2_slabs) / 2;
    float* const scratch = fold_scratch + (size_t)model * kFoldScratchFloats;
    const int n_out = kParamOut[jb.param], ldw = kParamIn[jb.param];
    const int tile = blockIdx.x;
    const int ot = tile / (kDwMaxXTiles + 1), xt = tile % (kDwMaxXTiles + 1);
    AdamCoef ac;
    if (A.state) ac = adam_coef(A.state[0] + 1.0f, A.lr, A.beta1, A.beta2);
    const GradEmit emit{A, ac, accumulate, model};
    if (ot < n_ot && xt == kDwMaxXTiles) {
        const int m = threadIdx.x;
        if (m < 32) {
            float sacc = 0.f;
            for (int sp = 0; sp < nsplit; ++sp) {
                const float* sl = slabs + (size_t)(s0 + sp) * kDwSlabFloats + (size_t)8 * kDwMaxXTiles * 64 * 16 +
                                  (fold >= 0 ? kDwFoldRow0 : ot) * 64;
                sacc += F8 ? sl[m] : sl[m] + sl[m + 32];
            }
            const int o = F8 ? 32 * ot + chain_feature(m >> 4, f8_row_h(m & 15), f8_row_j(m & 15)) : 32 * ot + m;
            if (o < n_out) {
                emit(G.b[jid] + o, sacc);
                if (jid % kNumDwJobs == kDwJobDir) scratch[kFoldS + o] = sacc;
            }
        }
    } else if (ot < n_ot && xt < n_xt) {
        const int e4 = threadIdx.x;
        const float4* src = reinterpret_cast<const float4*>(slabs + (size_t)s0 * kDwSlabFloats +
                                                            ((size_t)(fold >= 0 ? dw_fold_block(xt) : ot * kDwMaxXTiles + xt) * 64) * 16) + e4;
        float4 acc = make_float4(0.f, 0.f, 0.f, 0.f);
#pragma unroll 8
        for (int sp = 0; sp < nsplit; ++sp) {
            const float4 v = src[(size_t)sp * (kDwSlabFloats / 4)];
            acc.x += v.x; acc.y += v.y; acc.z += v.z; acc.w += v.w;
        }
        const int lane = e4 & 63, rq = e4 >> 6;
        const int h = lane >> 5, ncol = lane & 31;
        const int m0 = 8 * rq + 4 * h;
        const int o0 = F8 ? 32 * ot + chain_feature(m0 >> 4, f8_row_h(m0 & 15), f8_row_j(m0 & 15)) : 32 * ot + m0;
        const int xi = 32 * xt + ncol;
        int xs = xi >> 4;
        const int i = xi & 15;
        const int sh = F8 ? f8_row_h(i) : slab_nat_h(i), sj = F8 ? f8_row_j(i) : slab_nat_j(i);
        int enc, col0;
        if (xs < jb.x1_slabs) { enc = jb.x1_enc; col0 = jb.x1_col0; }
        else { xs -= jb.x1_slabs; enc = jb.x2_enc; col0 = jb.x2_col0; }
        int col;
        if (enc == 0 || enc == kDwEncFold) col = col0 + chain_feature(xs, sh, sj);
        else {
            const int ch = (enc == 1) ? xyz_slot_channel(xs, sh, sj) : dir_slot_channel(xs, sh, sj);
            col = ch < 0 ? -1 : col0 + ch;
        }
        if (enc == kDwEncFold) {
            const float vals[4] = {acc.x, acc.y, acc.z, acc.w};
#pragma unroll
            for (int k = 0; k < 4; ++k)
                if (o0 + k < n_out) scratch[kFoldG + (size_t)(o0 + k) * kW + col] = vals[k];
        } else if (col >= 0 && col < ldw) {
            const float vals[4] = {acc.x, acc.y, acc.z, acc.w};
#pragma unroll
            for (int k = 0; k < 4; ++k) {
                const int o = o0 + k;
                if (o < n_out) emit(G.w[jid] + (size_t)o * ldw + col, vals[k]);
            }
        }
    }
    if (A.state) {
        __syncthreads();
        if (threadIdx.x == 0) {
            unsigned* ticket = reinterpret_cast<unsigned*>(A.state + 1);
            const unsigned prev = atomicAdd(ticket, 1u);
            if (prev == gridDim.x * gridDim.y - 1) {
                *ticket = 0u;
                A.state[0] = A.state[0] + 1.0f;
            }
        }
    }
}

constexpr int kFoldBlocks = 32 + 64 + 1;
__global__ __launch_bounds__(256) void mlp_bwd_fold_kernel(FoldArgs F, const float* __restrict__ fold_scratch, int accumulate, AdamFused A) {
    constexpr int PA = 257, PB = 33;
    __shared__ float lds[2 * 32 * PA];
    __shared__ float part[4][16][64];
    const int model = blockIdx.y, bx = blockIdx.x, t = threadIdx.x;
    const int lane = t & 63, wave = t >> 6;
    const float* __restrict__ Gm = fold_scratch + (size_t)model * kFoldScratchFloats + kFoldG;
    const float* __restrict__ sv = fold_scratch + (size_t)model * kFoldScratchFloats + kFoldS;
    const float* __restrict__ Wf = F.image[model] + (size_t)kFoldWf * 256;
    const float* __restrict__ Wdx = F.image[model] + (size_t)kFoldWdx * 256;
    const float* __restrict__ bf = F.image[model] + (size_t)kFoldBf * 256;
    AdamCoef ac;
    if (A.state) ac = adam_coef(A.state[0], A.lr, A.beta1, A.beta2);
    const GradEmit emit{A, ac, accumulate, model};
    if (bx == kFoldBlocks - 1) {
        float a4[4] = {0.f, 0.f, 0.f, 0.f};
#pragma unroll 8
        for (int j = 0; j < 128; j += 4)
#pragma unroll
            for (int q = 0; q < 4; ++q) a4[q] = __builtin_fmaf(Wdx[(size_t)(j + q) * 256 + t], sv[j + q], a4[q]);
        emit(F.gb_final[model] + t, (a4[0] + a4[1]) + (a4[2] + a4[3]));
        return;
    }
    const bool dir = bx < 32;
    const int row0 = dir ? 32 * (bx >> 3) : 32 * ((bx - 32) >> 3), col0 = dir ? 32 * (bx & 7) : 32 * ((bx - 32) & 7);
    f32x16 acc;
#pragma unroll
    for (int r = 0; r < 16; ++r) acc[r] = 0.0f;
    const int m = lane & 31, kh = lane >> 5;
    if (dir) {
        float* sa = lds;
        float* sb = lds + 32 * PA;
        float4 va[8], vb[8];
#pragma unroll
        for (int i = 0; i < 8; ++i) {
            const int row = (t >> 6) + 4 * i;
            va[i] = reinterpret_cast<const float4*>(Gm + (size_t)(row0 + row) * 256)[t & 63];
            vb[i] = reinterpret_cast<const float4*>(Wf + (size_t)(col0 + row) * 256)[t & 63];
        }
#pragma unroll
        for (int i = 0; i < 8; ++i) {
            const int o = ((t >> 6) + 4 * i) * PA + 4 * (t & 63);
            sa[o] = va[i].x; sa[o + 1] = va[i].y; sa[o + 2] = va[i].z; sa[o + 3] = va[i].w;
            sb[o] = vb[i].x; sb[o + 1] = vb[i].y; sb[o + 2] = vb[i].z; sb[o + 3] = vb[i].w;
        }
        __syncthreads();
        const float* pa = sa + m * PA + 64 * wave + kh;
        const float* pb = sb + m * PA + 64 * wave + kh;
#pragma unroll 8
        for (int k = 0; k < 64; k += 2) acc = __builtin_amdgcn_mfma_f32_32x32x2f32(pa[k], pb[k], acc, 0, 0, 0);
    } else {
        float* sa = lds;
        float* sb = lds + 128 * PB;
        const int c = t & 31, r0 = t >> 5;
        float va[16], vb[16];
#pragma unroll
        for (int i = 0; i < 16; ++i) {
            va[i] = Wdx[(size_t)(r0 + 8 * i) * 256 + row0 + c];
            vb[i] = Gm[(size_t)(r0 + 8 * i) * 256 + col0 + c];
        }
#pragma unroll
        for (int i = 0; i < 16; ++i) {
            sa[(r0 + 8 * i) * PB + c] = va[i];
            sb[(r0 + 8 * i) * PB + c] = vb[i];
        }
        __syncthreads();
        const float* pa = sa + (32 * wave + kh) * PB + m;
        const float* pb = sb + (32 * wave + kh) * PB + m;
#pragma unroll 8
        for (int j = 0; j < 32; j += 2) acc = __builtin_amdgcn_mfma_f32_32x32x2f32(pa[j * PB], pb[j * PB], acc, 0, 0, 0);
    }
#pragma unroll
    for (int r = 0; r < 16; ++r) part[wave][r][lane] = acc[r];
    __syncthreads();
#pragma unroll
    for (int i = 0; i < 4; ++i) {
        const int r = wave + 4 * i;
        const float v = ((part[0][r][lane] + part[1][r][lane]) + part[2][r][lane]) + part[3][r][lane];
        const int row = row0 + (r & 3) + 8 * (r >> 2) + 4 * (lane >> 5), col = col0 + (lane & 31);
        if (dir) emit(F.gw_dir[model] + (size_t)row * kParamIn[9] + col, __builtin_fmaf(sv[row], bf[col], v));
        else emit(F.gw_final[model] + (size_t)row * 256 + col, v);
    }
}

void launch_reduce(bool f8, const DwJobTable& jt, const float* slabs, const GradTable& G, float* fold_scratch, int accumulate,
                   const AdamFused& A, hipStream_t s) {
    const dim3 rgrid(8 * (kDwMaxXTiles + 1), (unsigned)jt.njobs);
    if (f8) hipLaunchKernelGGL(mlp_bwd_reduce_kernel<true>, rgrid, dim3(256), 0, s, jt, slabs, G, fold_scratch, accumulate, A);
    else hipLaunchKernelGGL(mlp_bwd_reduce_kernel<false>, rgrid, dim3(256), 0, s, jt, slabs, G, fold_scratch, accumulate, A);
}
void launch_fold(const FoldArgs& F, const float* fold_scratch, int n_models, int accumulate, const AdamFused& A, hipStream_t s) {
    hipLaunchKernelGGL(mlp_bwd_fold_kernel, dim3(kFoldBlocks, (unsigned)n_models), dim3(256), 0, s, F, fold_scratch, accumulate, A);
}

}
```

nerf_pl_amd/csrc/mlp_device.h:

```cpp
#pragma once
#include <type_traits>

#include "common.h"
#include "mlp_layout.h"

#ifndef NERFHIP_STREAM_PROBE
#define NERFHIP_STREAM_PROBE 0
#endif

namespace nerfhip {
using namespace mlp;

constexpr int kStoreAux = 2;

typedef __attribute__((ext_vector_type(8))) __bf16 bf16x8;
typedef __attribute__((ext_vector_type(4))) __bf16 bf16x4;
typedef __attribute__((ext_vector_type(2))) __bf16 bf16x2;
typedef __attribute__((ext_vector_type(4))) short s16x4;
typedef __attribute__((ext_vector_type(2))) short s16x2;
typedef __attribute__((ext_vector_type(16))) float f32x16;
typedef __attribute__((ext_vector_type(8))) float f32x8;
typedef __attribute__((ext_vector_type(4))) float f32x4;
typedef __attribute__((ext_vector_type(4))) unsigned u32x4;
typedef __attribute__((ext_vector_type(2))) int i32x2;
typedef __attribute__((ext_vector_type(8))) int i32x8;

template <int PREC> struct PrecTraits;
template <> struct PrecTraits<NERFHIP_BF16> {
    using Slab = bf16x8;
    static constexpr int NW = 8, WPS = 2;
};
template <> struct PrecTraits<NERFHIP_F32> {
    using Slab = f32x8;
    static constexpr int NW = 4, WPS = 1;
};

__device__ __forceinline__ void make_slab(bf16x8& s, const float (&v)[8]) {
#pragma unroll
    for (int j = 0; j < 8; ++j) s[j] = (__bf16)v[j];
}
__device__ __forceinline__ void make_slab(f32x8& s, const float (&v)[8]) {
#pragma unroll
    for (int j = 0; j < 8; ++j) s[j] = v[j];
}

template <int B, int E, typename F>
__device__ __forceinline__ void static_for(F&& f) {
    if constexpr (B < E) {
        f(std::integral_constant<int, B>{});
        static_for<B + 1, E>(f);
    }
}

__device__ __forceinline__ void glds16_s(const void* sbase, unsigned voff, unsigned lds_dst) {
    unsigned keep;
    asm volatile(
        "s_mov_b32 %0, m0\n\ts_mov_b32 m0, %3\n\ts_nop 0\n\tglobal_load_lds_dwordx4 %1, %2\n\ts_mov_b32 m0, %0"
        : "=&s"(keep)
        : "v"(voff), "s"(sbase), "s"(lds_dst)
        : "memory");
}
__device__ __forceinline__ void glds16_nt(const void* gsrc, unsigned lds_dst) {
    unsigned keep;
    asm volatile(
        "s_mov_b32 %0, m0\n\ts_mov_b32 m0, %2\n\ts_nop 0\n\tglobal_load_lds_dwordx4 %1, off nt\n\ts_mov_b32 m0, %0"
        : "=&s"(keep)
        : "v"(gsrc), "s"(lds_dst)
        : "memory");
}
__device__ __forceinline__ void glds16_nt_masked(const void* gsrc, unsigned lds_dst, unsigned long long mask) {
    unsigned keep;
    unsigned long long keep_exec;
    asm volatile(
        "s_mov_b32 %0, m0\n\ts_mov_b64 %1, exec\n\ts_mov_b32 m0, %3\n\ts_mov_b64 exec, %4\n\tglobal_load_lds_dwordx4 %2, off nt\n\t"
        "s_mov_b64 exec, %1\n\ts_mov_b32 m0, %0"
        : "=&s"(keep), "=&s"(keep_exec)
        : "v"(gsrc), "s"(lds_dst), "s"(mask)
        : "memory");
}
__device__ __forceinline__ void glds4(const void* gsrc, unsigned lds_dst) {
    unsigned keep;
    asm volatile(
        "s_mov_b32 %0, m0\n\ts_mov_b32 m0, %2\n\ts_nop 0\n\tglobal_load_lds_dword %1, off\n\ts_mov_b32 m0, %0"
        : "=&s"(keep)
        : "v"(gsrc), "s"(lds_dst)
        : "memory");
}

template <int N>
__device__ __forceinline__ void wait_vm_barrier() {
    static_assert(N >= 0 && N <= 63, "vmcnt is a 6-bit counter");
    asm volatile("s_waitcnt vmcnt(%0) lgkmcnt(0)\n\ts_barrier" ::"n"(N) : "memory");
}
template <int N>
__device__ __forceinline__ void wait_vm() {
    asm volatile("s_waitcnt vmcnt(%0) lgkmcnt(0)" ::"n"(N) : "memory");
}
template <bool BARRIER>
__device__ __forceinline__ void wait_vm_counted(int n) {
#define NH_WB(N) case N: if constexpr (BARRIER) wait_vm_barrier<N>(); else wait_vm<N>(); break;
    switch (n < 0 ? 0 : (n > 48 ? 48 : (n <= 8 ? n : (n & ~3)))) {
        NH_WB(0) NH_WB(1) NH_WB(2) NH_WB(3) NH_WB(4) NH_WB(5) NH_WB(6) NH_WB(7) NH_WB(8)
        NH_WB(12) NH_WB(16) NH_WB(20) NH_WB(24) NH_WB(28) NH_WB(32) NH_WB(36) NH_WB(40) NH_WB(44) NH_WB(48)
        default: if constexpr (BARRIER) wait_vm_barrier<0>(); else wait_vm<0>(); break;
    }
#undef NH_WB
}

template <int NW_, int NCH_, bool COUNT_STORES>
struct RingStream {
    static constexpr int NW = NW_, NCH = NCH_;
    static constexpr int LPW = kChunkPieces / NW;
    const uint8_t* gsrc;
    unsigned voff;
    unsigned lds_base;
    int wave;
    int pending;
    int pending_prev;
#if NERFHIP_STREAM_PROBE
    unsigned pr_wait = 0, pr_bar = 0, pr_n = 0;
#endif

    __device__ __forceinline__ void issue_piece(int c, int k) const {
        const int piece = wave + k * NW;
        glds16_s(gsrc + ((size_t)c * kChunkPieces + piece) * kPieceBytes, voff,
                 lds_base + (unsigned)((c % kSlots) * kChunkBytes + piece * kPieceBytes));
    }
    __device__ __forceinline__ void issue_chunk(int c) const {
#pragma unroll
        for (int i = 0; i < LPW; ++i) issue_piece(c, i);
    }
    template <int G>
    __device__ __forceinline__ void at_piece() {
        if constexpr (G % kChunkPieces == 0) boundary(G / kChunkPieces);
    }
    __device__ __forceinline__ void boundary(int c) {
        if constexpr (COUNT_STORES) {
            const int n = (c + 1 < NCH ? LPW : 0) + pending + pending_prev;
            pending_prev = pending;
            pending = 0;
#if NERFHIP_STREAM_PROBE
            const unsigned t0 = (unsigned)__builtin_amdgcn_s_memrealtime();
            wait_vm_counted<false>(n);
            const unsigned t1 = (unsigned)__builtin_amdgcn_s_memrealtime();
            asm volatile("s_barrier" ::: "memory");
            const unsigned t2 = (unsigned)__builtin_amdgcn_s_memrealtime();
            pr_wait += t1 - t0; pr_bar += t2 - t1; pr_n += 1;
#else
            wait_vm_counted<true>(n);
#endif
        } else if (c + 1 < NCH) {
            wait_vm_barrier<LPW>();
        } else {
            wait_vm_barrier<0>();
        }
        if (c + 2 < NCH) issue_chunk(c + 2);
    }
};

template <typename Slab>
__device__ __forceinline__ void store_slab_b128(int& pending, __amdgpu_buffer_rsrc_t rsrc, const Slab& s, unsigned off) {
    const u32x4* src = reinterpret_cast<const u32x4*>(&s);
#pragma unroll
    for (int q = 0; q < (int)(sizeof(Slab) / 16); ++q) {
        __builtin_amdgcn_raw_buffer_store_b128(src[q], rsrc, off + 16 * q, 0, kStoreAux);
        pending += 1;
    }
}

__device__ __forceinline__ void dw_store_block(float* __restrict__ block, const f32x16& a, int lane) {
#pragma unroll
    for (int q = 0; q < 4; ++q)
        reinterpret_cast<float4*>(block)[64 * q + lane] = make_float4(a[4 * q], a[4 * q + 1], a[4 * q + 2], a[4 * q + 3]);
}
__device__ __forceinline__ unsigned shader_cycles() { return (unsigned)__builtin_amdgcn_s_memrealtime(); }

__device__ __forceinline__ bf16x8 load_frag_tr16(const char* pb, int tr_off, int tr_s0, int tr_s1, int q) {
    union { s16x4 h2[2]; bf16x8 v; } f;
    f.h2[0] = __builtin_amdgcn_ds_read_tr16_b64_v4i16((__attribute__((address_space(3))) s16x4*)(pb + tr_off + q * 512 + tr_s0));
    f.h2[1] = __builtin_amdgcn_ds_read_tr16_b64_v4i16((__attribute__((address_space(3))) s16x4*)(pb + tr_off + q * 512 + tr_s1));
    return f.v;
}

}
```

nerf_pl_amd/csrc/mlp_dw_plan.h:

```cpp
#pragma once
#include "mlp_bwd_dw.h"

constexpr int kPlanF32 = 0, kPlanBf16 = 1, kPlanBf16F8 = 2;

constexpr int kDwWgsF32 = 512, kDwWgsBf16 = 256, kDwWgsF8 = 256;

static int64_t act_tiles(int64_t n_points, int dtype) {
    const int64_t ppw = 32 * (dtype == kPlanF32 ? 4 : 8);
    return (n_points + ppw - 1) / ppw * (ppw / 32);
}

constexpr int kDwCostA = 150, kDwCostB = 45;
constexpr int kDwMinIters = 48;
static int dw_target_wgs(int dtype) { return dtype == kPlanBf16F8 ? kDwWgsF8 : dtype == kPlanBf16 ? kDwWgsBf16 : kDwWgsF32; }
static int dw_plan(const int64_t* n_points, int n_models, int dtype, nerfhip::DwJobTable* jt) {
    using namespace nerfhip;
    using namespace nerfhip::mlp;
    const int njobs = n_models * kNumDwJobs;
    int64_t units[kDwMaxJobs];
    int64_t cap[kDwMaxJobs];
    int ns[kDwMaxJobs];
    int64_t cost[kDwMaxJobs];
    int total = 0;
    for (int j = 0; j < njobs; ++j) {
        const int64_t tiles = act_tiles(n_points[j / kNumDwJobs], dtype);
        const DwJob& jb = kDwJobs[j % kNumDwJobs];
        const int ca = dtype == kPlanBf16 ? kDwCostA : 1;
        const int cb = dtype == kPlanBf16 ? kDwCostB : 0;
        cost[j] = ca + (int64_t)cb * (jb.dy_slabs + jb.x1_slabs + jb.x2_slabs + (j % kNumDwJobs == kDwJobDir ? 2 : 0));
        units[j] = tiles / (dtype == kPlanBf16F8 ? 2 : 1);
        cap[j] = units[j] / kDwMinIters;
        if (cap[j] < 1) cap[j] = 1;
        if (j % kNumDwJobs == kDwJobFinal || j % kNumDwJobs == kDwJobSigma) {
            cap[j] = 0;
            ns[j] = 0;
            continue;
        }
        ns[j] = 1;
        ++total;
    }
    const int target = dw_target_wgs(dtype);
    while (total < target) {
        int best = -1;
        for (int j = 0; j < njobs; ++j) {
            if (ns[j] >= cap[j]) continue;
            if (best < 0) { best = j; continue; }
            const int64_t a = units[j] * cost[j] * ns[best], b = units[best] * cost[best] * ns[j];
            const int jj = j % kNumDwJobs, bb = best % kNumDwJobs;
            const bool j_big = jj >= 1 && jj <= 7, b_big = bb >= 1 && bb <= 7;
            if (a > b || (a == b && j_big && !b_big)) best = j;
        }
        if (best < 0) break;
        ++ns[best];
        ++total;
    }
    if (jt) {
        int off = 0;
        for (int j = 0; j < kDwMaxJobs; ++j) {
            const int jj = j < njobs ? j : 0;
            jt->job[j] = kDwJobs[jj % kNumDwJobs];
            jt->nsplit[j] = j < njobs ? ns[j] : 0;
            jt->soff[j] = off;
            jt->ntiles[j] = act_tiles(n_points[jj / kNumDwJobs], dtype);
            jt->fold_of[j] = (j < njobs && ns[j] == 0 && j % kNumDwJobs == kDwJobSigma) ? j - kDwJobSigma + kDwJobDir : -1;
            if (j < njobs) off += ns[j];
        }
        jt->soff[kDwMaxJobs] = off;
        jt->njobs = njobs;
    }
    return total;
}
```

Before: 1.086 million.

## Fuse first-layer weight gradient into the bf16 backward chain kernel

For bf16, the backward chain kernel now computes the first MLP layer's weight and bias gradients itself. It stages the encoded xyz inputs in LDS, either recomputing the positional encoding from rays or DMA-loading it, and accumulates MFMA partials per workgroup over R blocks. It also skips the dy store for that layer. The separate dw job for layer 0 is dropped from the plan, and the reduce kernel sums the chain's per-workgroup partials. This removes one dy write/read round trip and a dw job, at the cost of using all of a CU's LDS in the chain kernel (lower occupancy) and adding extra partial-sum workspace.

```diff
diff --git a/include/nerfhip.h b/include/nerfhip.h
--- a/include/nerfhip.h
+++ b/include/nerfhip.h
@@ -127,6 +127,8 @@
 } nerfhip_adam_fused;
 size_t nerfhip_mlp_dw_workspace_bytes_multi(const int64_t* n_points_host, int n_models, int dtype);
 int nerfhip_mlp_dw_plan(const int64_t* n_points_host, int n_models, int dtype, int* splits_out, int* stage_kib_out);
+int nerfhip_mlp_dw_step_plan(const int64_t* n_points_host, int n_models, int dtype, int* splits_out, int* chain_out,
+                             size_t* layout_out);
 int nerfhip_mlp_bwd_multi(int n_models, const float* const* g_out_host, const float* const* out_host, const int64_t* n_host,
                           const void* const* packed_bwd_host, const void* const* acts_host, void* const* dys_host,
                           void* dw_workspace, float* const* grad_w_host, float* const* grad_b_host, int accumulate, int dtype,
diff --git a/nerf_pl_amd/_lib.py b/nerf_pl_amd/_lib.py
--- a/nerf_pl_amd/_lib.py
+++ b/nerf_pl_amd/_lib.py
@@ -90,6 +90,8 @@
                                ctypes.POINTER(_c_void_p), ctypes.POINTER(_c_void_p), _int, _int, _c_void_p],
     "nerfhip_mlp_dw_workspace_bytes_multi": [ctypes.POINTER(_i64), _int, _int],
     "nerfhip_mlp_dw_plan": [ctypes.POINTER(_i64), _int, _int, ctypes.POINTER(_int), ctypes.POINTER(_int)],
+    "nerfhip_mlp_dw_step_plan": [ctypes.POINTER(_i64), _int, _int, ctypes.POINTER(_int), ctypes.POINTER(_int),
+                                 ctypes.POINTER(ctypes.c_size_t)],
     "nerfhip_mlp_bwd_multi": [_int, ctypes.POINTER(_c_void_p), ctypes.POINTER(_c_void_p), ctypes.POINTER(_i64),
                               ctypes.POINTER(_c_void_p), ctypes.POINTER(_c_void_p), ctypes.POINTER(_c_void_p), _c_void_p,
                               ctypes.POINTER(_c_void_p), ctypes.POINTER(_c_void_p), _int, _int, _int, _c_void_p, _c_void_p, _c_void_p],
diff --git a/nerf_pl_amd/csrc/mlp_bwd.hip b/nerf_pl_amd/csrc/mlp_bwd.hip
--- a/nerf_pl_amd/csrc/mlp_bwd.hip
+++ b/nerf_pl_amd/csrc/mlp_bwd.hip
@@ -32,7 +32,26 @@
     if (!n_points_host || n_models < 1 || n_models > nerfhip::kDwMaxModels || !valid_dtype(dtype)) return 0;
     for (int m = 0; m < n_models; ++m)
         if (n_points_host[m] <= 0) return 0;
-    return dw_workspace_bytes(dw_plan(n_points_host, n_models, dtype, nullptr), n_models);
+    return dw_step_layout(n_points_host, n_models, dtype, nullptr, nullptr).total_floats * sizeof(float);
+}
+
+extern "C" int nerfhip_mlp_dw_step_plan(const int64_t* n_points_host, int n_models, int dtype, int* splits_out, int* chain_out,
+                                        size_t* layout_out) {
+    if (!n_points_host || !splits_out || !chain_out || !layout_out || n_models < 1 || n_models > nerfhip::kDwMaxModels || !valid_dtype(dtype))
+        return NERFHIP_E_BADARG;
+    for (int m = 0; m < n_models; ++m)
+        if (n_points_host[m] <= 0) return NERFHIP_E_BADARG;
+    nerfhip::DwJobTable jt;
+    nerfhip::ChainDw1 dw1;
+    const DwStepLayout L = dw_step_layout(n_points_host, n_models, dtype, &jt, &dw1);
+    for (int j = 0; j < n_models * nerfhip::mlp::kNumDwJobs; ++j) splits_out[j] = jt.nsplit[j];
+    chain_out[0] = dw1.count[0] > 0 ? dw1.R : 0;
+    for (int m = 0; m < nerfhip::kDwMaxModels; ++m) chain_out[1 + m] = dw1.count[m];
+    layout_out[0] = L.fold_off * sizeof(float);
+    layout_out[1] = L.part_off * sizeof(float);
+    layout_out[2] = (size_t)dw1.stride * sizeof(float);
+    layout_out[3] = L.total_floats * sizeof(float);
+    return L.nwg;
 }
 
 extern "C" int nerfhip_mlp_dw_plan(const int64_t* n_points_host, int n_models, int dtype, int* splits_out, int* stage_kib_out) {
@@ -63,11 +82,11 @@
                                       grad_b_host, accumulate, dtype, phases, g_scale, adam, nullptr, stream);
 }
 
-extern "C" int nerfhip_mlp_bwd_multi_rays(int n_models, const float* const* g_out_host, const float* const* out_host,
-                                          const int64_t* n_host, const void* const* packed_bwd_host, const void* const* acts_host,
-                                          void* const* dys_host, void* dw_workspace, float* const* grad_w_host,
-                                          float* const* grad_b_host, int accumulate, int dtype, int phases, const float* g_scale,
-                                          const nerfhip_adam_fused* adam, const nerfhip_enc_source* enc, nerfhip_stream_t stream) {
+static int bwd_multi_impl(int n_models, const float* const* g_out_host, const float* const* out_host,
+                          const int64_t* n_host, const void* const* packed_bwd_host, const void* const* acts_host,
+                          void* const* dys_host, void* dw_workspace, float* const* grad_w_host,
+                          float* const* grad_b_host, int accumulate, int dtype, int phases, const float* g_scale,
+                          const nerfhip_adam_fused* adam, const nerfhip_enc_source* enc, bool step, nerfhip_stream_t stream) {
     NERFHIP_CHECK_ARG(n_models >= 1 && n_models <= nerfhip::kDwMaxModels);
     if (!valid_dtype(dtype)) return NERFHIP_E_UNSUPPORTED;
     bool regen[nerfhip::kDwMaxModels] = {false, false};
@@ -92,14 +111,25 @@
              ((uintptr_t)dys_host[m])) & 15)
             return NERFHIP_E_ALIGN;
     }
-    const int nwg = dw_plan(n_host, n_models, dtype, &jt);
+    nerfhip::ChainDw1 dw1 = {};
+    int nwg;
+    float* fold_scratch;
+    if (step) {
+        const DwStepLayout L = dw_step_layout(n_host, n_models, dtype, &jt, &dw1);
+        nwg = L.nwg;
+        fold_scratch = (float*)dw_workspace + L.fold_off;
+        dw1.part = (float*)dw_workspace + L.part_off;
+    } else {
+        nwg = dw_plan(n_host, n_models, dtype, &jt);
+        fold_scratch = (float*)dw_workspace + (size_t)nwg * nerfhip::mlp::kDwSlabFloats;
+    }
+    const bool chain_dw1 = dw1.count[0] > 0;
     for (int m = 0; m < nerfhip::kDwMaxModels; ++m) {
         const bool on = m < n_models && regen[m];
-        jt.enc_rays[m] = on ? enc->rays[m] : nullptr;
-        jt.enc_z[m] = on ? enc->z[m] : nullptr;
-        jt.enc_tpr[m] = on ? enc->S[m] / 32 : 1;
-    }
-    float* const fold_scratch = (float*)dw_workspace + (size_t)nwg * nerfhip::mlp::kDwSlabFloats;
+        jt.enc_rays[m] = dw1.enc_rays[m] = on ? enc->rays[m] : nullptr;
+        jt.enc_z[m] = dw1.enc_z[m] = on ? enc->z[m] : nullptr;
+        jt.enc_tpr[m] = dw1.enc_tpr[m] = on ? enc->S[m] / 32 : 1;
+    }
     nerfhip::FoldArgs F;
     for (int m = 0; m < nerfhip::kDwMaxModels; ++m) {
         const int mm = m < n_models ? m : 0;
@@ -134,7 +164,8 @@
     if (do_chain) {
         int64_t tiles[nerfhip::kDwMaxModels];
         for (int m = 0; m < n_models; ++m) tiles[m] = act_tiles(n_host[m], dtype);
-        nerfhip::launch_bwd_chain(n_models, g_out_host, g_scale, out_host, n_host, packed_bwd_host, acts_host, dys_host, dtype, tiles, s);
+        if (chain_dw1) nerfhip::launch_bwd_chain_dw1(n_models, g_out_host, g_scale, out_host, n_host, packed_bwd_host, acts_host, dys_host, dw1, s);
+        else nerfhip::launch_bwd_chain(n_models, g_out_host, g_scale, out_host, n_host, packed_bwd_host, acts_host, dys_host, dtype, tiles, s);
     }
     if (do_dw) {
         if (dtype == NERFHIP_BF16_F8) nerfhip::launch_dw_f8(jt, (float*)dw_workspace, nwg, s);
@@ -144,10 +175,19 @@
 #endif
     }
     if (do_reduce) {
-        nerfhip::launch_reduce(dtype == NERFHIP_BF16_F8, jt, (const float*)dw_workspace, G, fold_scratch, accumulate, A, s);
+        nerfhip::launch_reduce(dtype == NERFHIP_BF16_F8, jt, (const float*)dw_workspace, G, fold_scratch, accumulate, A, dw1, s);
         nerfhip::launch_fold(F, (const float*)fold_scratch, n_models, accumulate, A, s);
     }
     return nerfhip_launch_status();
+}
+
+extern "C" int nerfhip_mlp_bwd_multi_rays(int n_models, const float* const* g_out_host, const float* const* out_host,
+                                          const int64_t* n_host, const void* const* packed_bwd_host, const void* const* acts_host,
+                                          void* const* dys_host, void* dw_workspace, float* const* grad_w_host,
+                                          float* const* grad_b_host, int accumulate, int dtype, int phases, const float* g_scale,
+                                          const nerfhip_adam_fused* adam, const nerfhip_enc_source* enc, nerfhip_stream_t stream) {
+    return bwd_multi_impl(n_models, g_out_host, out_host, n_host, packed_bwd_host, acts_host, dys_host, dw_workspace, grad_w_host,
+                          grad_b_host, accumulate, dtype, phases, g_scale, adam, enc, true, stream);
 }
 
 #if NERFHIP_DW_PROBE
@@ -165,8 +205,8 @@
     NERFHIP_CHECK_ARG(grad_w_host && grad_b_host);
     for (int i = 0; i < 12; ++i) NERFHIP_CHECK_ARG(grad_w_host[i] && grad_b_host[i]);
     if (n == 0) return 0;
-    return nerfhip_mlp_bwd_multi(1, &g_out, &out, &n, &packed_bwd, &acts, &dys, dw_workspace, grad_w_host, grad_b_host, accumulate,
-                                 dtype, phases, nullptr, nullptr, stream);
+    return bwd_multi_impl(1, &g_out, &out, &n, &packed_bwd, &acts, &dys, dw_workspace, grad_w_host, grad_b_host, accumulate,
+                          dtype, phases, nullptr, nullptr, nullptr, false, stream);
 }
 
 extern "C" int nerfhip_mlp_bwd(const float* g_out, const float* out, int64_t n, const void* packed_bwd, const void* acts,
diff --git a/nerf_pl_amd/csrc/mlp_bwd_chain.h b/nerf_pl_amd/csrc/mlp_bwd_chain.h
--- a/nerf_pl_amd/csrc/mlp_bwd_chain.h
+++ b/nerf_pl_amd/csrc/mlp_bwd_chain.h
@@ -1,6 +1,8 @@
 #pragma once
 #include <hip/hip_runtime.h>
 #include <stdint.h>
+
+#include "mlp_bwd_dw.h"
 
 namespace nerfhip {
 struct BwdChainArgs {
@@ -15,4 +17,6 @@
 void launch_bwd_chain(int n_models, const float* const* g_out, const float* g_scale, const float* const* out, const int64_t* n,
                       const void* const* packed_bwd, const void* const* acts, void* const* dys, int dtype, const int64_t* tiles,
                       hipStream_t s);
+void launch_bwd_chain_dw1(int n_models, const float* const* g_out, const float* g_scale, const float* const* out, const int64_t* n,
+                          const void* const* packed_bwd, const void* const* acts, void* const* dys, const ChainDw1& dw1, hipStream_t s);
 }
diff --git a/nerf_pl_amd/csrc/mlp_bwd_chain.hip b/nerf_pl_amd/csrc/mlp_bwd_chain.hip
--- a/nerf_pl_amd/csrc/mlp_bwd_chain.hip
+++ b/nerf_pl_amd/csrc/mlp_bwd_chain.hip
@@ -46,7 +46,7 @@
     return m;
 }
 
-template <int PREC, int L, int NT, int NKS, bool MASK, bool F8, int IN_PAIRS, typename Slab>
+template <int PREC, int L, int NT, int NKS, bool MASK, bool F8, int IN_PAIRS, bool STORE = true, typename Slab>
 __device__ __forceinline__ int run_bwd_layer_tm(BwdStream<PREC>& st, const unsigned lds_lo, const unsigned lds_hi, const unsigned sig_lds,
                                                 const Slab (&gin)[NKS - kBwdLayers[L].sigma_slab], Slab* out,
                                                 __amdgpu_buffer_rsrc_t acts, int gate_off, int mask_piece,
@@ -159,7 +159,7 @@
             make_slab(out[2 * t + sl], v8);
         }
         }
-        if constexpr (!F8) {
+        if constexpr (!F8 && STORE) {
             __amdgpu_buffer_rsrc_t dys_l = __builtin_amdgcn_make_buffer_rsrc(dy_tile + (size_t)dy_sec * 64 * sizeof(Slab) * act_il(PREC), 0,
                                                                               (int)(2 * NT * 64 * sizeof(Slab) * act_il(PREC)), 0x00020000);
             constexpr int TB = kChainBurst / 2 > 0 ? kChainBurst / 2 : 1;
@@ -178,9 +178,15 @@
     return 127;
 }
 
-template <int PREC, bool F8>
-__global__ __launch_bounds__(PrecTraits<PREC>::NW * 64, PrecTraits<PREC>::WPS)
-void mlp_bwd_chain_kernel(BwdChainArgs A, const float* __restrict__ g_scale) {
+constexpr int kDw1Ex = 2 * kChunkBytes, kDw1X = kDw1Ex + 4 * 16 * kPieceBytes;
+constexpr int kDw1LdsBytes = kDw1X + 8 * kXyzSlabs * kPieceBytes;
+static_assert(kSlots == 3 && kDw1Ex + 2 * 16 * kPieceBytes == kSlots * kChunkBytes, "the exchange region starts with ring slot 2");
+static_assert(bwd_chunks(NERFHIP_BF16) % kSlots == 1, "the W^T stream's last chunk lies in ring slot 0");
+static_assert(kDw1LdsBytes == 160 * 1024, "the DW1 chain uses the whole LDS of a CU");
+
+template <int PREC, bool F8, bool DW1>
+__device__ __forceinline__ void bwd_chain_body(const BwdChainArgs& A, const float* __restrict__ g_scale, const ChainDw1& D) {
+    static_assert(!DW1 || (PREC == NERFHIP_BF16 && !F8), "DW1 is the bf16-storing chain's variant");
     const int mdl = ((int)blockIdx.x >= A.blocks0) ? 1 : 0;
     const unsigned wg = blockIdx.x - (mdl ? (unsigned)A.blocks0 : 0u);
     const float* __restrict__ g_out = mdl ? A.g_out[1] : A.g_out[0];
@@ -195,14 +201,29 @@
     constexpr int kGateOff = F8 ? f8_act_gate_off() : act_mask_off(PREC);
     constexpr int kDyTile = F8 ? f8_dy_tile_bytes() : kDySlabs * 64 * (int)sizeof(Slab);
     constexpr int NW = PrecTraits<PREC>::NW;
-    __shared__ __attribute__((aligned(1024))) char ring[kSlots * kChunkBytes + NW * 64 * (int)sizeof(Slab)];
+    __shared__ __attribute__((aligned(1024))) char ring[DW1 ? kDw1LdsBytes : kSlots * kChunkBytes + NW * 64 * (int)sizeof(Slab)];
 #if NERFHIP_STREAM_PROBE
     const uint64_t probe_t0 = __builtin_amdgcn_s_memrealtime();
 #endif
     const int lane = threadIdx.x & 63;
     const int wave = __builtin_amdgcn_readfirstlane((int)(threadIdx.x >> 6));
     const int h = lane >> 5;
-    const int64_t tile = (int64_t)wg * NW + wave;
+    [[maybe_unused]] f32x16 acc1[2];
+    [[maybe_unused]] float db1a = 0.0f, db1b = 0.0f;
+    int nblk = 1;
+    if constexpr (DW1) {
+#pragma unroll
+        for (int x = 0; x < 2; ++x)
+#pragma unroll
+            for (int r = 0; r < 16; ++r) acc1[x][r] = 0.0f;
+        const int left = (mdl ? D.blocks[1] : D.blocks[0]) - (int)wg * D.R;
+        nblk = left < D.R ? left : D.R;
+    }
+    [[maybe_unused]] const float* __restrict__ enc_rays = DW1 ? (mdl ? D.enc_rays[1] : D.enc_rays[0]) : nullptr;
+    [[maybe_unused]] const float* __restrict__ enc_z = DW1 ? (mdl ? D.enc_z[1] : D.enc_z[0]) : nullptr;
+    [[maybe_unused]] const int enc_tpr = DW1 ? (mdl ? D.enc_tpr[1] : D.enc_tpr[0]) : 1;
+    for (int blk = 0; blk < nblk; ++blk) {
+    const int64_t tile = ((int64_t)wg * (DW1 ? D.R : 1) + blk) * NW + wave;
     const int64_t p = tile * 32 + (lane & 31);
     const bool valid = p < n;
     const int64_t pc = valid ? p : n - 1;
@@ -229,6 +250,33 @@
     st.wave = wave;
     st.pending = 0;
     st.pending_prev = 0;
+    if constexpr (DW1) {
+        int ln = lane;
+        asm volatile("" : "+v"(ln));
+        const int n32 = ln & 31, hx = ln >> 5;
+        if (enc_rays) {
+            const float zv = enc_z[tile * 32 + n32];
+            const float* __restrict__ rp = enc_rays + (size_t)((unsigned)tile / (unsigned)enc_tpr) * 8;
+            float xv[3];
+#pragma unroll
+            for (int c = 0; c < 3; ++c) xv[c] = nh_add(rp[c], nh_mul(rp[3 + c], zv));
+#pragma unroll
+            for (int ks = 0; ks < kXyzSlabs; ++ks) {
+                const bf16x8 e = dw_encode_slab<10, kXyzSlabs>(xv, hx, ks);
+                const int unit = (2 * n32 + hx) ^ ((ks & 1) ? 8 : 0);
+                *reinterpret_cast<bf16x8*>(ring + kDw1X + (wave * kXyzSlabs + ks) * kPieceBytes + unit * 16) = e;
+            }
+        } else {
+            const uint8_t* xsrc = acts_base + tile_block_off(tile, kActTile, IL) + (size_t)kActEncX * kPieceBytes * IL;
+            const int dma_off_even = ((ln & 1) * 32 + (ln >> 1)) * 16, dma_off_odd = ((ln & 1) * 32 + ((ln ^ 8) >> 1)) * 16;
+#pragma unroll
+            for (int ks = 0; ks < kXyzSlabs; ++ks) {
+                const unsigned dst = (unsigned)__builtin_amdgcn_readfirstlane(
+                    (int)((unsigned)(uintptr_t)ring + (unsigned)(kDw1X + (wave * kXyzSlabs + ks) * kPieceBytes)));
+                glds16(xsrc + (size_t)ks * kPieceBytes * IL + ((ks & 1) ? dma_off_odd : dma_off_even), dst);
+            }
+        }
+    }
     st.issue_chunk(0);
     st.issue_chunk(1);
     const unsigned lds_lo = (unsigned)(uintptr_t)ring + (unsigned)lane * 16u;
@@ -300,7 +348,47 @@
         st.pending_prev = 0;
         st.gsrc = gsrc0;
     }
+    if constexpr (DW1) {
+        sb = run_bwd_layer_tm<PREC, 8, 8, 16, true, F8, 8, false>(st, lds_lo, lds_hi, sig_lds, reinterpret_cast<const Slab(&)[16]>(gb), ga, acts, kGateOff,
+                                                                  mask_piece_h(1), dys, dy_tile, dy_h(1), f8_dy_section(dy_h(1)), dy_h(2), sb, lane);
+        int ln = lane;
+        asm volatile("" : "+v"(ln));
+        const int n32 = ln & 31;
+        const int unit_even = (2 * n32 + (ln >> 5)) * 16, unit_odd = ((2 * n32 + (ln >> 5)) ^ 8) * 16;
+        auto put_tile = [&](int buf_off) {
+            static_for<0, 16>([&](auto sc) {
+                constexpr int s = decltype(sc)::value;
+                *reinterpret_cast<bf16x8*>(ring + buf_off + s * kPieceBytes + ((s & 1) ? unit_odd : unit_even)) = ga[s];
+            });
+        };
+        const int grp = ln >> 4, c = ln & 15;
+        const int tr_off = (grp & 1) * kPieceBytes + (2 * (8 * (grp >> 1) + (c >> 2)) + ((c & 3) & 1)) * 16 + ((c & 3) >> 1) * 8;
+        const int tr_s0 = (grp & 1) ? 128 : 0, tr_s1 = 128 - tr_s0;
+#pragma clang loop unroll(disable)
+        for (int r = 0; r < 2; ++r) {
+            asm volatile("s_waitcnt lgkmcnt(0)\n\ts_barrier" ::: "memory");
+            if ((wave >> 2) == r) put_tile(kDw1Ex + (wave & 3) * 16 * kPieceBytes);
+            asm volatile("s_waitcnt lgkmcnt(0)\n\ts_barrier" ::: "memory");
+#pragma unroll
+            for (int tt = 0; tt < 4; ++tt) {
+                const char* dyb = ring + kDw1Ex + (tt * 16 + 2 * wave) * kPieceBytes;
+                const char* xb = ring + kDw1X + (4 * r + tt) * kXyzSlabs * kPieceBytes;
+                const bf16x8 a0 = load_frag_tr16(dyb, tr_off, tr_s0, tr_s1, 0), b00 = load_frag_tr16(xb, tr_off, tr_s0, tr_s1, 0),
+                             b10 = load_frag_tr16(xb + 2 * kPieceBytes, tr_off, tr_s0, tr_s1, 0);
+                const bf16x8 a1 = load_frag_tr16(dyb, tr_off, tr_s0, tr_s1, 1), b01 = load_frag_tr16(xb, tr_off, tr_s0, tr_s1, 1),
+                             b11 = load_frag_tr16(xb + 2 * kPieceBytes, tr_off, tr_s0, tr_s1, 1);
+                acc1[0] = __builtin_amdgcn_mfma_f32_32x32x16_bf16(a0, b00, acc1[0], 0, 0, 0);
+                acc1[1] = __builtin_amdgcn_mfma_f32_32x32x16_bf16(a0, b10, acc1[1], 0, 0, 0);
+                acc1[0] = __builtin_amdgcn_mfma_f32_32x32x16_bf16(a1, b01, acc1[0], 0, 0, 0);
+                acc1[1] = __builtin_amdgcn_mfma_f32_32x32x16_bf16(a1, b11, acc1[1], 0, 0, 0);
+                dw_bias_sum(a0, db1a, db1b);
+                dw_bias_sum(a1, db1a, db1b);
+            }
+        }
+        asm volatile("s_waitcnt lgkmcnt(0)\n\ts_barrier" ::: "memory");
+    } else {
     NH_BWD(8, gb, ga, 0)
+    }
 #undef NH_BWD
     if constexpr (F8 && PREC == NERFHIP_BF16) {
 #pragma unroll
@@ -313,6 +401,35 @@
         pr[3] = (unsigned)(__builtin_amdgcn_s_memrealtime() - probe_t0);
     }
 #endif
+    }
+    if constexpr (DW1) {
+        float* const part = D.part + (size_t)blockIdx.x * (size_t)D.stride;
+        __amdgpu_buffer_rsrc_t prs = __builtin_amdgcn_make_buffer_rsrc(part, 0, kChainDw1Floats * (int)sizeof(float), 0x00020000);
+        int pend = 0;
+        int ln = lane;
+        asm volatile("" : "+v"(ln));
+#pragma unroll
+        for (int x = 0; x < 2; ++x)
+#pragma unroll
+            for (int q = 0; q < 4; ++q) {
+                const f32x4 v = {acc1[x][4 * q], acc1[x][4 * q + 1], acc1[x][4 * q + 2], acc1[x][4 * q + 3]};
+                store_slab_b128(pend, prs, v, (unsigned)(((wave * 2 + x) * 1024 + (64 * q + ln) * 4) * (int)sizeof(float)));
+            }
+        float db = db1a + db1b;
+        db += __shfl_xor(db, 32);
+        if (ln < 32) part[8 * 2 * 1024 + wave * 32 + ln] = db;
+    }
+}
+
+template <int PREC, bool F8>
+__global__ __launch_bounds__(PrecTraits<PREC>::NW * 64, PrecTraits<PREC>::WPS)
+void mlp_bwd_chain_kernel(BwdChainArgs A, const float* __restrict__ g_scale) {
+    const ChainDw1 none = {};
+    bwd_chain_body<PREC, F8, false>(A, g_scale, none);
+}
+__global__ __launch_bounds__(PrecTraits<NERFHIP_BF16>::NW * 64, PrecTraits<NERFHIP_BF16>::WPS)
+void mlp_bwd_chain_dw1_kernel(BwdChainArgs A, const float* __restrict__ g_scale, ChainDw1 D) {
+    bwd_chain_body<NERFHIP_BF16, false, true>(A, g_scale, D);
 }
 
 
@@ -339,4 +456,18 @@
     else
         hipLaunchKernelGGL((mlp_bwd_chain_kernel<NERFHIP_F32, false>), dim3(blocks), dim3(256), 0, s, A, g_scale);
 }
-}
+
+void launch_bwd_chain_dw1(int n_models, const float* const* g_out, const float* g_scale, const float* const* out, const int64_t* n,
+                          const void* const* packed_bwd, const void* const* acts, void* const* dys, const ChainDw1& dw1, hipStream_t s) {
+    BwdChainArgs A;
+    for (int m = 0; m < 2; ++m) {
+        const int mm = m < n_models ? m : 0;
+        A.g_out[m] = g_out[mm]; A.out[m] = out[mm]; A.n[m] = n[mm];
+        A.packed_bwd[m] = (const uint8_t*)packed_bwd[mm]; A.acts[m] = (const uint8_t*)acts[mm]; A.dys[m] = (uint8_t*)dys[mm];
+    }
+    A.blocks0 = dw1.count[0];
+    unsigned wgs = 0;
+    for (int m = 0; m < n_models; ++m) wgs += (unsigned)dw1.count[m];
+    hipLaunchKernelGGL(mlp_bwd_chain_dw1_kernel, dim3(wgs), dim3(512), 0, s, A, g_scale, dw1);
+}
+}
diff --git a/nerf_pl_amd/csrc/mlp_bwd_dw.h b/nerf_pl_amd/csrc/mlp_bwd_dw.h
--- a/nerf_pl_amd/csrc/mlp_bwd_dw.h
+++ b/nerf_pl_amd/csrc/mlp_bwd_dw.h
@@ -35,6 +35,20 @@
 constexpr int kDwFoldStageSlabs = 28;
 constexpr int kDwFoldSigmaSlab = 26;
 
+constexpr int kChainDw1Floats = 8 * 2 * 1024 + 8 * 32;
+constexpr int kChainDw1MaxR = 4;
+struct ChainDw1 {
+    float* part;
+    int stride;
+    int R;
+    int first[kDwMaxModels];
+    int count[kDwMaxModels];
+    int blocks[kDwMaxModels];
+    const float* enc_rays[kDwMaxModels];
+    const float* enc_z[kDwMaxModels];
+    int enc_tpr[kDwMaxModels];
+};
+
 struct GradTable {
     float* w[kDwMaxJobs];
     float* b[kDwMaxJobs];
@@ -59,7 +73,7 @@
 void launch_dw(int prec, const DwJobTable& jt, float* slabs, int nwg, hipStream_t s);
 void launch_dw_f8(const DwJobTable& jt, float* slabs, int nwg, hipStream_t s);
 void launch_reduce(bool f8, const DwJobTable& jt, const float* slabs, const GradTable& G, float* fold_scratch, int accumulate,
-                   const AdamFused& A, hipStream_t s);
+                   const AdamFused& A, const ChainDw1& dw1, hipStream_t s);
 void launch_fold(const FoldArgs& F, const float* fold_scratch, int n_models, int accumulate, const AdamFused& A, hipStream_t s);
 #if NERFHIP_DW_PROBE
 int read_dw_probe(unsigned* host_dst, int n_words);
diff --git a/nerf_pl_amd/csrc/mlp_bwd_dw.hip b/nerf_pl_amd/csrc/mlp_bwd_dw.hip
--- a/nerf_pl_amd/csrc/mlp_bwd_dw.hip
+++ b/nerf_pl_amd/csrc/mlp_bwd_dw.hip
@@ -30,47 +30,6 @@
     return d > kDwMaxDepth ? kDwMaxDepth : d;
 }
 
-__device__ __forceinline__ void dw_bias_sum(const bf16x8& a, float& s0, float& s1) {
-    const bf16x2 one = {(__bf16)1.0f, (__bf16)1.0f};
-    s0 = __builtin_amdgcn_fdot2_f32_bf16(bf16x2{a[0], a[1]}, one, s0, false);
-    s1 = __builtin_amdgcn_fdot2_f32_bf16(bf16x2{a[2], a[3]}, one, s1, false);
-    s0 = __builtin_amdgcn_fdot2_f32_bf16(bf16x2{a[4], a[5]}, one, s0, false);
-    s1 = __builtin_amdgcn_fdot2_f32_bf16(bf16x2{a[6], a[7]}, one, s1, false);
-}
-
-template <int F, int SLABS>
-__device__ __forceinline__ bf16x8 dw_encode_slab(const float (&v)[3], int h, int ks) {
-    constexpr int NPAIR = 3 * (F / 2);
-    constexpr float kInv2PiHi = 0.15915494f, kInv2PiLo = 6.4206297e-9f;
-    float rh[3], rl[3];
-#pragma unroll
-    for (int c = 0; c < 3; ++c) {
-        const float vs = h ? 2.0f * v[c] : v[c];
-        rh[c] = vs * kInv2PiHi;
-        rl[c] = __builtin_fmaf(vs, kInv2PiHi, -rh[c]) + vs * kInv2PiLo;
-    }
-    bf16x8 out;
-#pragma unroll
-    for (int q = 0; q < 4; ++q) {
-        const int p = 4 * ks + q;
-        float s, co;
-        if (p < NPAIR) {
-            const int i = p / 3, c = p - 3 * i;
-            const float sc = (float)(1 << (2 * i));
-            const float rhc = c == 0 ? rh[0] : (c == 1 ? rh[1] : rh[2]), rlc = c == 0 ? rl[0] : (c == 1 ? rl[1] : rl[2]);
-            const float t = __builtin_amdgcn_fractf(rhc * sc) + rlc * sc;
-            s = __builtin_amdgcn_sinf(t);
-            co = __builtin_amdgcn_cosf(t);
-        } else {
-            const int tail = 2 * (p - NPAIR);
-            s = (tail == 0) ? (h ? v[2] : v[0]) : 0.0f;
-            co = (tail == 0) ? (h ? 0.0f : v[1]) : 0.0f;
-        }
-        out[2 * q] = (__bf16)s;
-        out[2 * q + 1] = (__bf16)co;
-    }
-    return out;
-}
 
 template <int PREC>
 __global__ __launch_bounds__(512, 2)
diff --git a/nerf_pl_amd/csrc/mlp_bwd_reduce.hip b/nerf_pl_amd/csrc/mlp_bwd_reduce.hip
--- a/nerf_pl_amd/csrc/mlp_bwd_reduce.hip
+++ b/nerf_pl_amd/csrc/mlp_bwd_reduce.hip
@@ -20,7 +20,7 @@
 
 template <bool F8>
 __global__ __launch_bounds__(256) void mlp_bwd_reduce_kernel(DwJobTable jobs, const float* __restrict__ slabs, GradTable G,
-                                                              float* __restrict__ fold_scratch, int accumulate, AdamFused A) {
+                                                              float* __restrict__ fold_scratch, int accumulate, AdamFused A, ChainDw1 dw1) {
     const int jid = blockIdx.y;
     const DwJob jb = jobs.job[jid];
     const int model = jid / kNumDwJobs;
@@ -35,7 +35,54 @@
     AdamCoef ac;
     if (A.state) ac = adam_coef(A.state[0] + 1.0f, A.lr, A.beta1, A.beta2);
     const GradEmit emit{A, ac, accumulate, model};
-    if (ot < n_ot && xt == kDwMaxXTiles) {
+    const int n_part = (jid % kNumDwJobs == 0) ? dw1.count[model] : 0;
+    if (n_part > 0) {
+        __shared__ float4 red[4][64];
+        const float* const part0 = dw1.part + (size_t)dw1.first[model] * (size_t)dw1.stride;
+        const int t = threadIdx.x;
+        if (tile < 64) {
+            const int blk = tile >> 2, e4 = 64 * (tile & 3) + (t & 63), grp = t >> 6;
+            const int per = (n_part + 3) / 4, p0 = grp * per, p1 = (p0 + per < n_part) ? p0 + per : n_part;
+            const float* src = part0 + (size_t)blk * 1024 + (size_t)e4 * 4;
+            float4 acc = make_float4(0.f, 0.f, 0.f, 0.f);
+#pragma unroll 8
+            for (int p = p0; p < p1; ++p) {
+                const float4 v = *reinterpret_cast<const float4*>(src + (size_t)p * (size_t)dw1.stride);
+                acc.x += v.x; acc.y += v.y; acc.z += v.z; acc.w += v.w;
+            }
+            red[grp][t & 63] = acc;
+            __syncthreads();
+            if (grp == 0) {
+                const float4 r0 = red[0][t], r1 = red[1][t], r2 = red[2][t], r3 = red[3][t];
+                const float vals[4] = {((r0.x + r1.x) + r2.x) + r3.x, ((r0.y + r1.y) + r2.y) + r3.y, ((r0.z + r1.z) + r2.z) + r3.z,
+                                       ((r0.w + r1.w) + r2.w) + r3.w};
+                const int lane = e4 & 63, rq = e4 >> 6;
+                const int o0 = 32 * (blk >> 1) + 8 * rq + 4 * (lane >> 5);
+                const int xi = 32 * (blk & 1) + (lane & 31);
+                const int ch = xyz_slot_channel(xi >> 4, slab_nat_h(xi & 15), slab_nat_j(xi & 15));
+                if (ch >= 0 && ch < ldw) {
+#pragma unroll
+                    for (int k = 0; k < 4; ++k) emit(G.w[jid] + (size_t)(o0 + k) * ldw + ch, vals[k]);
+                }
+            }
+        } else if (tile < 72) {
+            const int m = t & 31, grp = t >> 5;
+            const int per = (n_part + 7) / 8, p0 = grp * per, p1 = (p0 + per < n_part) ? p0 + per : n_part;
+            const float* src = part0 + 8 * 2 * 1024 + (tile - 64) * 32 + m;
+            float sacc = 0.f;
+#pragma unroll 8
+            for (int p = p0; p < p1; ++p) sacc += src[(size_t)p * (size_t)dw1.stride];
+            float* const redf = reinterpret_cast<float*>(&red[0][0]);
+            redf[t] = sacc;
+            __syncthreads();
+            if (t < 32) {
+                float v = redf[t];
+#pragma unroll
+                for (int g = 1; g < 8; ++g) v += redf[32 * g + t];
+                emit(G.b[jid] + 32 * (tile - 64) + t, v);
+            }
+        }
+    } else if (ot < n_ot && xt == kDwMaxXTiles) {
         const int m = threadIdx.x;
         if (m < 32) {
             float sacc = 0.f;
@@ -190,10 +237,10 @@
 }
 
 void launch_reduce(bool f8, const DwJobTable& jt, const float* slabs, const GradTable& G, float* fold_scratch, int accumulate,
-                   const AdamFused& A, hipStream_t s) {
+                   const AdamFused& A, const ChainDw1& dw1, hipStream_t s) {
     const dim3 rgrid(8 * (kDwMaxXTiles + 1), (unsigned)jt.njobs);
-    if (f8) hipLaunchKernelGGL(mlp_bwd_reduce_kernel<true>, rgrid, dim3(256), 0, s, jt, slabs, G, fold_scratch, accumulate, A);
-    else hipLaunchKernelGGL(mlp_bwd_reduce_kernel<false>, rgrid, dim3(256), 0, s, jt, slabs, G, fold_scratch, accumulate, A);
+    if (f8) hipLaunchKernelGGL(mlp_bwd_reduce_kernel<true>, rgrid, dim3(256), 0, s, jt, slabs, G, fold_scratch, accumulate, A, dw1);
+    else hipLaunchKernelGGL(mlp_bwd_reduce_kernel<false>, rgrid, dim3(256), 0, s, jt, slabs, G, fold_scratch, accumulate, A, dw1);
 }
 void launch_fold(const FoldArgs& F, const float* fold_scratch, int n_models, int accumulate, const AdamFused& A, hipStream_t s) {
     hipLaunchKernelGGL(mlp_bwd_fold_kernel, dim3(kFoldBlocks, (unsigned)n_models), dim3(256), 0, s, F, fold_scratch, accumulate, A);
diff --git a/nerf_pl_amd/csrc/mlp_device.h b/nerf_pl_amd/csrc/mlp_device.h
--- a/nerf_pl_amd/csrc/mlp_device.h
+++ b/nerf_pl_amd/csrc/mlp_device.h
@@ -64,6 +64,14 @@
     unsigned keep;
     asm volatile(
         "s_mov_b32 %0, m0\n\ts_mov_b32 m0, %2\n\ts_nop 0\n\tglobal_load_lds_dwordx4 %1, off nt\n\ts_mov_b32 m0, %0"
+        : "=&s"(keep)
+        : "v"(gsrc), "s"(lds_dst)
+        : "memory");
+}
+__device__ __forceinline__ void glds16(const void* gsrc, unsigned lds_dst) {
+    unsigned keep;
+    asm volatile(
+        "s_mov_b32 %0, m0\n\ts_mov_b32 m0, %2\n\ts_nop 0\n\tglobal_load_lds_dwordx4 %1, off\n\ts_mov_b32 m0, %0"
         : "=&s"(keep)
         : "v"(gsrc), "s"(lds_dst)
         : "memory");
@@ -182,4 +190,46 @@
     return f.v;
 }
 
-}
+__device__ __forceinline__ void dw_bias_sum(const bf16x8& a, float& s0, float& s1) {
+    const bf16x2 one = {(__bf16)1.0f, (__bf16)1.0f};
+    s0 = __builtin_amdgcn_fdot2_f32_bf16(bf16x2{a[0], a[1]}, one, s0, false);
+    s1 = __builtin_amdgcn_fdot2_f32_bf16(bf16x2{a[2], a[3]}, one, s1, false);
+    s0 = __builtin_amdgcn_fdot2_f32_bf16(bf16x2{a[4], a[5]}, one, s0, false);
+    s1 = __builtin_amdgcn_fdot2_f32_bf16(bf16x2{a[6], a[7]}, one, s1, false);
+}
+
+template <int F, int SLABS>
+__device__ __forceinline__ bf16x8 dw_encode_slab(const float (&v)[3], int h, int ks) {
+    constexpr int NPAIR = 3 * (F / 2);
+    constexpr float kInv2PiHi = 0.15915494f, kInv2PiLo = 6.4206297e-9f;
+    float rh[3], rl[3];
+#pragma unroll
+    for (int c = 0; c < 3; ++c) {
+        const float vs = h ? 2.0f * v[c] : v[c];
+        rh[c] = vs * kInv2PiHi;
+        rl[c] = __builtin_fmaf(vs, kInv2PiHi, -rh[c]) + vs * kInv2PiLo;
+    }
+    bf16x8 out;
+#pragma unroll
+    for (int q = 0; q < 4; ++q) {
+        const int p = 4 * ks + q;
+        float s, co;
+        if (p < NPAIR) {
+            const int i = p / 3, c = p - 3 * i;
+            const float sc = (float)(1 << (2 * i));
+            const float rhc = c == 0 ? rh[0] : (c == 1 ? rh[1] : rh[2]), rlc = c == 0 ? rl[0] : (c == 1 ? rl[1] : rl[2]);
+            const float t = __builtin_amdgcn_fractf(rhc * sc) + rlc * sc;
+            s = __builtin_amdgcn_sinf(t);
+            co = __builtin_amdgcn_cosf(t);
+        } else {
+            const int tail = 2 * (p - NPAIR);
+            s = (tail == 0) ? (h ? v[2] : v[0]) : 0.0f;
+            co = (tail == 0) ? (h ? 0.0f : v[1]) : 0.0f;
+        }
+        out[2 * q] = (__bf16)s;
+        out[2 * q + 1] = (__bf16)co;
+    }
+    return out;
+}
+
+}
diff --git a/nerf_pl_amd/csrc/mlp_dw_plan.h b/nerf_pl_amd/csrc/mlp_dw_plan.h
--- a/nerf_pl_amd/csrc/mlp_dw_plan.h
+++ b/nerf_pl_amd/csrc/mlp_dw_plan.h
@@ -1,4 +1,6 @@
 #pragma once
+#include <stddef.h>
+
 #include "mlp_bwd_dw.h"
 
 constexpr int kPlanF32 = 0, kPlanBf16 = 1, kPlanBf16F8 = 2;
@@ -13,7 +15,7 @@
 constexpr int kDwCostA = 150, kDwCostB = 45;
 constexpr int kDwMinIters = 48;
 static int dw_target_wgs(int dtype) { return dtype == kPlanBf16F8 ? kDwWgsF8 : dtype == kPlanBf16 ? kDwWgsBf16 : kDwWgsF32; }
-static int dw_plan(const int64_t* n_points, int n_models, int dtype, nerfhip::DwJobTable* jt) {
+static int dw_plan(const int64_t* n_points, int n_models, int dtype, nerfhip::DwJobTable* jt, bool drop_first = false) {
     using namespace nerfhip;
     using namespace nerfhip::mlp;
     const int njobs = n_models * kNumDwJobs;
@@ -31,7 +33,7 @@
         units[j] = tiles / (dtype == kPlanBf16F8 ? 2 : 1);
         cap[j] = units[j] / kDwMinIters;
         if (cap[j] < 1) cap[j] = 1;
-        if (j % kNumDwJobs == kDwJobFinal || j % kNumDwJobs == kDwJobSigma) {
+        if (j % kNumDwJobs == kDwJobFinal || j % kNumDwJobs == kDwJobSigma || (drop_first && j % kNumDwJobs == 0)) {
             cap[j] = 0;
             ns[j] = 0;
             continue;
@@ -70,3 +72,39 @@
     }
     return total;
 }
+
+#ifndef NERFHIP_CHAIN_DW1_R
+#define NERFHIP_CHAIN_DW1_R 4
+#endif
+constexpr int kChainDw1R = NERFHIP_CHAIN_DW1_R;
+static_assert(kChainDw1R >= 1 && kChainDw1R <= nerfhip::kChainDw1MaxR, "blocks per DW1 chain workgroup");
+struct DwStepLayout {
+    int nwg;
+    size_t fold_off;
+    size_t part_off;
+    size_t total_floats;
+};
+static bool dw_step_uses_chain_dw1(int dtype) { return dtype == kPlanBf16; }
+static DwStepLayout dw_step_layout(const int64_t* n_points, int n_models, int dtype, nerfhip::DwJobTable* jt, nerfhip::ChainDw1* dw1) {
+    using namespace nerfhip;
+    const bool on = dw_step_uses_chain_dw1(dtype);
+    DwStepLayout L;
+    L.nwg = dw_plan(n_points, n_models, dtype, jt, on);
+    L.fold_off = (size_t)L.nwg * mlp::kDwSlabFloats;
+    L.part_off = L.fold_off + (size_t)n_models * mlp::kFoldScratchFloats;
+    int parts = 0;
+    ChainDw1 d = {};
+    d.stride = kChainDw1Floats;
+    d.R = kChainDw1R;
+    for (int m = 0; m < kDwMaxModels; ++m) {
+        d.enc_tpr[m] = 1;
+        if (!on || m >= n_models) continue;
+        d.blocks[m] = (int)(act_tiles(n_points[m], dtype) / 8);
+        d.first[m] = parts;
+        d.count[m] = (d.blocks[m] + d.R - 1) / d.R;
+        parts += d.count[m];
+    }
+    L.total_floats = L.part_off + (size_t)parts * kChainDw1Floats;
+    if (dw1) *dw1 = d;
+    return L;
+}
```

New measurement: 1.079 million. No clear change (-0.6%).
